# chlhnu/DOT-SOCP

Hardware: AMD Instinct MI355X
Metric: ADMM iters/sec on NxNxT dot2d staggered grid at 1/2/4/8 MI355X (higher is better)
Workload: dtype f64

## Files before the change

dot-socp_amd/capi.py:

```python
import ctypes
import os

import numpy as np

_HERE = os.path.dirname(os.path.abspath(__file__))
LIB_PATH = os.path.join(_HERE, "lib", "libdotsocp.so")

i64 = ctypes.c_longlong
dbl = ctypes.c_double
vp = ctypes.c_void_p


class DotsocpError(RuntimeError):
    def __init__(self, code, msg):
        super().__init__(f"libdotsocp error {code}: {msg}")
        self.code = code


class Problem(ctypes.Structure):
    _fields_ = [("dim", ctypes.c_int), ("weighted", ctypes.c_int),
                ("ny", i64), ("nx", i64), ("nt", i64),
                ("D", dbl), ("E", dbl), ("cScale", dbl), ("dScale", dbl),
                ("normc", dbl), ("normd", dbl)]


class Opts(ctypes.Structure):
    _fields_ = [("tau", dbl), ("sigma", dbl), ("tol", dbl), ("maxit", i64),
                ("ifCheckStepByStep", ctypes.c_int), ("checkPrimDualFeas", ctypes.c_int),
                ("scaling", ctypes.c_int), ("time_limit", dbl)]


class Result(ctypes.Structure):
    _fields_ = [("sigma", dbl), ("sigma_internal", dbl), ("cScale", dbl), ("dScale", dbl),
                ("times", dbl * 7), ("iters", i64), ("hist_len", i64), ("stopped", ctypes.c_int),
                ("time_extra", dbl)]


class AccOpts(ctypes.Structure):
    _fields_ = [("restart", i64), ("rho", dbl), ("theta", dbl)]


REPORT_BINS = 49
REPORT_RHO_FLOOR = 1e-8


class Report(ctypes.Structure):
    _fields_ = [("n_nodes", i64), ("n_cells", i64), ("mass_err", dbl), ("neg_err", dbl),
                ("rho_min", dbl), ("rho_neg", i64), ("rho_hist", i64 * REPORT_BINS),
                ("fq_max", dbl), ("fq_pos", i64), ("fq_hist", i64 * REPORT_BINS),
                ("cost", dbl), ("nonfinite", i64)]


class AdvectOpts(ctypes.Structure):
    _fields_ = [("n", i64), ("nsub", ctypes.c_int), ("direction", ctypes.c_int), ("rho_floor", dbl)]


class PushOpts(ctypes.Structure):
    _fields_ = [("n", i64), ("nsub", ctypes.c_int), ("direction", ctypes.c_int), ("rho_floor", dbl), ("nf", i64)]


class MapReport(ctypes.Structure):
    _fields_ = [("n", i64), ("n_clamped", i64), ("n_still", i64), ("mass", dbl),
                ("cost_map", dbl), ("cost_length", dbl), ("cost_action", dbl), ("disp_mean", dbl), ("len_mean", dbl),
                ("disp_max", dbl), ("len_max", dbl), ("detour_max", dbl),
                ("detour_hist", i64 * REPORT_BINS), ("detour_over", i64)]


class RenderOpts(ctypes.Structure):
    _fields_ = [("mode", ctypes.c_int), ("channels", ctypes.c_int), ("nf", i64), ("nlevels", ctypes.c_int),
                ("barrier_index", ctypes.c_int), ("vmax", dbl), ("skip_y", i64), ("skip_x", i64), ("mask_frac", dbl)]


class RenderInfo(ctypes.Structure):
    _fields_ = [("vmax", dbl), ("rho_min", dbl), ("nonfinite", i64), ("masked", i64), ("my", i64), ("mx", i64)]


RENDER_LINEAR, RENDER_INVERTED, RENDER_LEVELS = 0, 1, 2
METHOD_INPALM, METHOD_PALM, METHOD_ACCADMM = 0, 1, 2


F_PHI, F_Q, F_ALPHA, F_Z, F_BETA, F_C, F_WEIGHT = range(7)

SYMBOLS = {
    "dotsocp_last_error": (ctypes.c_char_p, []),
    "dotsocp_version": (ctypes.c_char_p, []),
    "dotsocp_device_count": (ctypes.c_int, []),
    "dotsocp_proj_soc": (ctypes.c_int, [vp, vp, i64, i64]),
    "dotsocp_bfd": (ctypes.c_int, [vp, vp, i64, i64, i64, dbl, dbl]),
    "dotsocp_bfd_conj": (ctypes.c_int, [vp, vp, i64, i64, i64, dbl]),
    "dotsocp_bfd1d": (ctypes.c_int, [vp, vp, i64, i64, dbl, dbl]),
    "dotsocp_bfd_conj1d": (ctypes.c_int, [vp, vp, i64, i64, dbl]),
    "dotsocp_oper_poisson": (ctypes.c_int, [vp, vp, i64, i64, i64, dbl]),
    "dotsocp_dctn": (ctypes.c_int, [vp, i64, i64, i64, ctypes.c_int]),
    "dotsocp_proj_soc_dev": (ctypes.c_int, [vp, vp, i64, i64, vp]),
    "dotsocp_bfd_dev": (ctypes.c_int, [vp, vp, i64, i64, i64, dbl, dbl, vp]),
    "dotsocp_bfd_conj_dev": (ctypes.c_int, [vp, vp, i64, i64, i64, dbl, vp]),
    "dotsocp_create": (vp, [ctypes.POINTER(Problem), ctypes.c_int, ctypes.c_int]),
    "dotsocp_create_multi": (vp, [ctypes.POINTER(Problem), ctypes.c_int, ctypes.c_int]),
    "dotsocp_destroy": (None, [vp]),
    "dotsocp_rccl_unique_id": (ctypes.c_int, [vp]),
    "dotsocp_attach_rccl": (ctypes.c_int, [vp, vp, ctypes.c_int, ctypes.c_int]),
    "dotsocp_slab_range": (ctypes.c_int, [i64, ctypes.c_int, ctypes.c_int, ctypes.POINTER(i64), ctypes.POINTER(i64)]),
    "dotsocp_field_len": (i64, [ctypes.POINTER(Problem), ctypes.c_int]),
    "dotsocp_dct_algorithm": (ctypes.c_int, [i64]),
    "dotsocp_dct_levels": (ctypes.c_int, [i64, ctypes.c_int]),
    "dotsocp_cdft_levels": (ctypes.c_int, [i64]),
    "dotsocp_tsolve_tri_safe": (ctypes.c_int, [i64, i64, i64]),
    "dotsocp_cone_writes_beta": (ctypes.c_int, [i64, dbl, i64, ctypes.c_int, ctypes.c_int, ctypes.c_int, dbl, dbl]),
    "dotsocp_rescale_due": (ctypes.c_int, [i64, ctypes.c_int, dbl, dbl]),
    "dotsocp_qcone_form": (ctypes.c_int, [i64, dbl, i64, ctypes.c_int, ctypes.c_int, ctypes.c_int, ctypes.c_int, dbl, dbl]),
    "dotsocp_release_cache": (i64, []),
    "dotsocp_upload": (ctypes.c_int, [vp, ctypes.c_int, vp]),
    "dotsocp_upload_layers": (ctypes.c_int, [vp, ctypes.c_int, vp, i64, i64]),
    "dotsocp_download": (ctypes.c_int, [vp, ctypes.c_int, vp]),
    "dotsocp_begin": (ctypes.c_int, [vp, ctypes.POINTER(Opts)]),
    "dotsocp_begin_method": (ctypes.c_int, [vp, ctypes.POINTER(Opts), ctypes.c_int, ctypes.POINTER(AccOpts)]),
    "dotsocp_run": (ctypes.c_int, [vp, i64, ctypes.POINTER(i64)]),
    "dotsocp_recover_outputs": (ctypes.c_int, [vp, vp, vp, vp, vp, vp, vp, vp, vp]),
    "dotsocp_report_edges": (ctypes.c_int, [vp]),
    "dotsocp_solution_report": (ctypes.c_int, [vp, vp, vp, ctypes.POINTER(Report), vp, vp]),
    "dotsocp_recover_velocity": (ctypes.c_int, [vp, vp, vp, dbl, vp, vp]),
    "dotsocp_advect_particles": (ctypes.c_int, [vp, vp, vp, ctypes.POINTER(AdvectOpts), vp, vp, vp, vp, ctypes.POINTER(i64)]),
    "dotsocp_push_mass": (ctypes.c_int, [vp, vp, vp, ctypes.POINTER(PushOpts), vp, vp, vp, vp, vp, ctypes.POINTER(i64),
                                         ctypes.POINTER(dbl), vp]),
    "dotsocp_map_report": (ctypes.c_int, [vp, vp, vp, ctypes.POINTER(AdvectOpts), vp, vp, vp, ctypes.POINTER(MapReport),
                                          vp, vp, vp]),
    "dotsocp_render_evolution": (ctypes.c_int, [vp, vp, vp, ctypes.POINTER(RenderOpts), vp, vp, vp, vp, vp, vp, vp,
                                                ctypes.POINTER(RenderInfo)]),
    "dotsocp_jump_next_level": (ctypes.c_int, [vp, vp]),
    "dotsocp_finish": (ctypes.c_int, [vp, ctypes.POINTER(Result)]),
    "dotsocp_get_history": (ctypes.c_int, [vp, vp, vp, vp, vp]),
    "dotsocp_set_profiling": (ctypes.c_int, [vp, ctypes.c_int]),
    "dotsocp_kernel_time": (ctypes.c_int, [vp, ctypes.c_char_p, ctypes.POINTER(dbl), ctypes.POINTER(i64)]),
    "dotsocp_canary_check": (ctypes.c_int, []),
    "dotsocp_poisson_phi": (ctypes.c_int, [vp]),
    "dotsocp_synchronize": (ctypes.c_int, [vp]),
    "dotsocp_weights_create": (vp, [ctypes.c_int, i64, i64, i64, ctypes.c_int]),
    "dotsocp_weights_destroy": (None, [vp]),
    "dotsocp_weights_len": (i64, [i64, i64, i64, ctypes.c_int, ctypes.c_int]),
    "dotsocp_weights_set": (ctypes.c_int, [vp, vp]),
    "dotsocp_weights_set_space": (ctypes.c_int, [vp, vp, vp]),
    "dotsocp_weights_restrict": (ctypes.c_int, [vp, ctypes.c_int]),
    "dotsocp_weights_log10_mean": (ctypes.c_int, [vp, ctypes.c_int, ctypes.POINTER(dbl)]),
    "dotsocp_weights_download": (ctypes.c_int, [vp, ctypes.c_int, vp]),
    "dotsocp_upload_weight_from": (ctypes.c_int, [vp, vp, ctypes.c_int]),
}

_lib = None


def _share_torchs_hip_runtime():
    import importlib.util
    import sys
    if "torch" in sys.modules or os.environ.get("DOTSOCP_SYSTEM_HIP"):
        return
    try:
        spec = importlib.util.find_spec("torch")
    except (ImportError, ValueError):
        return
    if not spec or not spec.submodule_search_locations:
        return
    for name in ("libamdhip64.so", "libamdhip64.so.7"):
        path = os.path.join(list(spec.submodule_search_locations)[0], "lib", name)
        if os.path.exists(path):
            try:
                ctypes.CDLL(path, mode=ctypes.RTLD_GLOBAL)
            except OSError:
                pass
            return


def lib():
    global _lib
    if _lib is None:
        _share_torchs_hip_runtime()
        if not os.path.exists(LIB_PATH):
            raise ImportError(
                f"{LIB_PATH} is missing: build the HIP extension first "
                "(python -c 'import __graft_entry__ as g; g.build()'); there is no CPU fallback")
        L = ctypes.CDLL(LIB_PATH)
        for name, (res, args) in SYMBOLS.items():
            f = getattr(L, name)
            f.restype = res
            f.argtypes = args
        _lib = L
    return _lib


def check(code):
    if code != 0:
        raise DotsocpError(code, lib().dotsocp_last_error().decode())


def fptr(a):
    if not isinstance(a, np.ndarray) or a.dtype != np.float64 or not (a.flags.f_contiguous or a.flags.c_contiguous):
        raise ValueError("expected a contiguous float64 numpy array")
    return a.ctypes.data


def slab_range(nt, world, rank):
    t0, t1 = i64(), i64()
    check(lib().dotsocp_slab_range(nt, world, rank, ctypes.byref(t0), ctypes.byref(t1)))
    return t0.value, t1.value


def rccl_unique_id():
    buf = (ctypes.c_ubyte * 128)()
    check(lib().dotsocp_rccl_unique_id(buf))
    return bytes(buf)


DCT_ALGORITHMS = ("none", "fft", "pfa", "rader", "bluestein", "dense")


def dct_algorithm(n):
    return DCT_ALGORITHMS[lib().dotsocp_dct_algorithm(int(n))]


def dct_levels(n, axis):
    return int(lib().dotsocp_dct_levels(int(n), int(axis)))


def cdft_levels(n):
    return int(lib().dotsocp_cdft_levels(int(n)))
```

dot-socp_amd/csrc/capi.hip:

```cpp
#include <cstring>
#include <new>

#include "comm.h"
#include "solver.h"
#include "weights.h"

using namespace dotsocp;

namespace dotsocp {
extern thread_local std::string g_last_error;
int dotsocp_slab_range_impl(i64 nt, int world, int rank, i64 *t0, i64 *t1);
}

struct dotsocp_ctx {
    Solver s;
};

struct dotsocp_weights {
    Weights w;
};

static int require_device() {
    int n = 0;
    if (hipGetDeviceCount(&n) != hipSuccess || n <= 0) {
        set_error("no HIP device available (libdotsocp has no CPU fallback)");
        return DOTSOCP_ENODEVICE;
    }
    return 0;
}

struct DevBuf {
    double *p = nullptr;
    ~DevBuf() { dfree(p); }
    int alloc(i64 n) { return dmalloc(&p, n); }
};

extern "C" {

const char *dotsocp_last_error(void) { return g_last_error.c_str(); }
const char *dotsocp_version(void) { return "dotsocp-mi355x 0.1 (gfx950)"; }

int dotsocp_device_count(void) {
    int n = 0;
    if (hipGetDeviceCount(&n) != hipSuccess) return 0;
    return n;
}

int dotsocp_proj_soc_dev(double *d_out, const double *d_in, dotsocp_i64 M, dotsocp_i64 K, void *stream) {
    DS_ARG(M >= 0 && K >= 2, "mexProjSoc needs an M x K matrix with K >= 2");
    DS_ARG(d_out && d_in, "NULL pointer");
    return launch_proj_soc(d_out, d_in, M, K, (hipStream_t)stream);
}

static int make_grid(Grid &g, i64 nt, i64 nx, i64 ny) {
    DS_ARG(nt >= 2 && nx >= 1 && ny >= 1, "need nt >= 2, nx >= 1, ny >= 1");
    g.set(ny, nx, nt, 0, nt);
    return 0;
}

int dotsocp_bfd_dev(double *d_z, const double *d_q, dotsocp_i64 nt, dotsocp_i64 nx, dotsocp_i64 ny, double scale,
                    double dF, void *stream) {
    Grid g;
    DS_CHECK(make_grid(g, nt, nx, ny));
    DS_ARG(d_z && d_q, "NULL pointer");
    return launch_bfd(g, d_z, d_q, scale, dF, (hipStream_t)stream);
}

int dotsocp_bfd_conj_dev(double *d_q, const double *d_z, dotsocp_i64 nt, dotsocp_i64 nx, dotsocp_i64 ny,
                         double scale, void *stream) {
    Grid g;
    DS_CHECK(make_grid(g, nt, nx, ny));
    DS_ARG(d_z && d_q, "NULL pointer");
    return launch_bfd_conj(g, d_q, d_z, scale, (hipStream_t)stream);
}

int dotsocp_proj_soc(double *out, const double *in, dotsocp_i64 M, dotsocp_i64 K) {
    DS_ARG(M >= 0 && K >= 2, "mexProjSoc needs an M x K matrix with K >= 2");
    if (M == 0) return 0;
    DS_ARG(out && in, "NULL pointer");
    DS_CHECK(require_device());
    DevBuf a, b;
    DS_CHECK(a.alloc(M * K));
    DS_CHECK(b.alloc(M * K));
    DS_HIP(hipMemcpy(a.p, in, sizeof(double) * M * K, hipMemcpyHostToDevice));
    DS_CHECK(launch_proj_soc(b.p, a.p, M, K, nullptr));
    DS_HIP(hipDeviceSynchronize());
    DS_HIP(hipMemcpy(out, b.p, sizeof(double) * M * K, hipMemcpyDeviceToHost));
    return 0;
}

int dotsocp_bfd(double *z, const double *q, dotsocp_i64 nt, dotsocp_i64 nx, dotsocp_i64 ny, double scale,
                double dF) {
    Grid g;
    DS_CHECK(make_grid(g, nt, nx, ny));
    DS_ARG(z && q, "NULL pointer");
    DS_CHECK(require_device());
    DevBuf dz, dq;
    DS_CHECK(dz.alloc(10 * g.Nz));
    DS_CHECK(dq.alloc(g.NqAlloc));
    DS_HIP(hipMemcpy(dz.p, z, sizeof(double) * 10 * g.Nz, hipMemcpyHostToDevice));
    DS_HIP(hipMemcpy(dq.p, q, sizeof(double) * g.NqAlloc, hipMemcpyHostToDevice));
    DS_CHECK(launch_bfd(g, dz.p, dq.p, scale, dF, nullptr));
    DS_HIP(hipDeviceSynchronize());
    DS_HIP(hipMemcpy(z, dz.p, sizeof(double) * 10 * g.Nz, hipMemcpyDeviceToHost));
    return 0;
}

int dotsocp_bfd_conj(double *q, const double *z, dotsocp_i64 nt, dotsocp_i64 nx, dotsocp_i64 ny, double scale) {
    Grid g;
    DS_CHECK(make_grid(g, nt, nx, ny));
    DS_ARG(z && q, "NULL pointer");
    DS_CHECK(require_device());
    DevBuf dz, dq;
    DS_CHECK(dz.alloc(10 * g.Nz));
    DS_CHECK(dq.alloc(g.NqAlloc));
    DS_HIP(hipMemcpy(dz.p, z, sizeof(double) * 10 * g.Nz, hipMemcpyHostToDevice));
    DS_CHECK(launch_bfd_conj(g, dq.p, dz.p, scale, nullptr));
    DS_HIP(hipDeviceSynchronize());
    DS_HIP(hipMemcpy(q, dq.p, sizeof(double) * g.NqAlloc, hipMemcpyDeviceToHost));
    return 0;
}

static const int k1dCols[6] = {0, 5, 6, 7, 8, 9};

int dotsocp_bfd1d(double *z, const double *q, dotsocp_i64 nt, dotsocp_i64 nx, double scale, double dF) {
    Grid g;
    DS_CHECK(make_grid(g, nt, 1, nx));
    DS_ARG(z && q, "NULL pointer");
    DS_CHECK(require_device());
    DevBuf dz, dq;
    DS_CHECK(dz.alloc(10 * g.Nz));
    DS_CHECK(dq.alloc(g.NqAlloc));
    for (int j = 0; j < 6; ++j)
        DS_HIP(hipMemcpy(dz.p + k1dCols[j] * g.Nz, z + j * g.Nz, sizeof(double) * g.Nz, hipMemcpyHostToDevice));
    DS_HIP(hipMemcpy(dq.p, q, sizeof(double) * g.NqAlloc, hipMemcpyHostToDevice));
    DS_CHECK(launch_bfd(g, dz.p, dq.p, scale, dF, nullptr));
    DS_HIP(hipDeviceSynchronize());
    for (int j = 0; j < 6; ++j)
        DS_HIP(hipMemcpy(z + j * g.Nz, dz.p + k1dCols[j] * g.Nz, sizeof(double) * g.Nz, hipMemcpyDeviceToHost));
    return 0;
}

int dotsocp_bfd_conj1d(double *q, const double *z, dotsocp_i64 nt, dotsocp_i64 nx, double scale) {
    Grid g;
    DS_CHECK(make_grid(g, nt, 1, nx));
    DS_ARG(z && q, "NULL pointer");
    DS_CHECK(require_device());
    DevBuf dz, dq;
    DS_CHECK(dz.alloc(10 * g.Nz));
    DS_CHECK(dq.alloc(g.NqAlloc));
    DS_HIP(hipMemset(dz.p, 0, sizeof(double) * 10 * g.Nz));
    for (int j = 0; j < 6; ++j)
        DS_HIP(hipMemcpy(dz.p + k1dCols[j] * g.Nz, z + j * g.Nz, sizeof(double) * g.Nz, hipMemcpyHostToDevice));
    DS_CHECK(launch_bfd_conj(g, dq.p, dz.p, scale, nullptr));
    DS_HIP(hipDeviceSynchronize());
    DS_HIP(hipMemcpy(q, dq.p, sizeof(double) * g.NqAlloc, hipMemcpyDeviceToHost));
    return 0;
}

static int dctn_dev(double *a, double *b, i64 ny, i64 nx, i64 nt, int inverse, DctPlan *py, DctPlan *px, DctPlan *pt) {
    if (!inverse) {
        DS_CHECK(launch_dct_axis(py, a, b, ny, nx, nt, 0, 0, nullptr));
        DS_CHECK(launch_dct_axis(px, b, a, ny, nx, nt, 1, 0, nullptr));
        DS_CHECK(launch_dct_axis(pt, a, b, ny, nx, nt, 2, 0, nullptr));
    } else {
        DS_CHECK(launch_dct_axis(pt, a, b, ny, nx, nt, 2, 1, nullptr));
        DS_CHECK(launch_dct_axis(px, b, a, ny, nx, nt, 1, 1, nullptr));
        DS_CHECK(launch_dct_axis(py, a, b, ny, nx, nt, 0, 1, nullptr));
    }
    return 0;
}

struct Plans {
    DctPlan *py = nullptr, *px = nullptr, *pt = nullptr;
    ~Plans() { dct_plan_destroy(py); dct_plan_destroy(px); dct_plan_destroy(pt); }
    int make(i64 ny, i64 nx, i64 nt) {
        DS_CHECK(dct_length_check(ny)); DS_CHECK(dct_length_check(nx)); DS_CHECK(dct_length_check(nt));
        py = dct_plan_create(ny); px = dct_plan_create(nx); pt = dct_plan_create(nt);
        if (!py || !px || !pt) { set_error("DCT plan allocation failed"); return DOTSOCP_EHIP; }
        return 0;
    }
};

int dotsocp_dctn(double *a, dotsocp_i64 ny, dotsocp_i64 nx, dotsocp_i64 nt, int inverse) {
    DS_ARG(a && ny >= 1 && nx >= 1 && nt >= 1, "bad array");
    DS_CHECK(dct_length_check(ny)); DS_CHECK(dct_length_check(nx)); DS_CHECK(dct_length_check(nt));
    DS_CHECK(require_device());
    const i64 n = ny * nx * nt;
    DevBuf da, db;
    Plans pl;
    DS_CHECK(da.alloc(n));
    DS_CHECK(db.alloc(n));
    DS_CHECK(pl.make(ny, nx, nt));
    DS_HIP(hipMemcpy(da.p, a, sizeof(double) * n, hipMemcpyHostToDevice));
    DS_CHECK(dctn_dev(da.p, db.p, ny, nx, nt, inverse, pl.py, pl.px, pl.pt));
    DS_HIP(hipDeviceSynchronize());
    DS_HIP(hipMemcpy(a, db.p, sizeof(double) * n, hipMemcpyDeviceToHost));
    return 0;
}

int dotsocp_oper_poisson(double *res, const double *rhs, dotsocp_i64 ny, dotsocp_i64 nx, dotsocp_i64 nt,
                         double kernelScale) {
    DS_ARG(res && rhs && ny >= 1 && nx >= 1 && nt >= 1, "bad array");
    DS_CHECK(dct_length_check(ny)); DS_CHECK(dct_length_check(nx)); DS_CHECK(dct_length_check(nt));
    DS_CHECK(require_device());
    const i64 n = ny * nx * nt;
    DevBuf da, db, cy, cx, ct;
    Plans pl;
    DS_CHECK(da.alloc(n));
    DS_CHECK(db.alloc(n));
    DS_CHECK(pl.make(ny, nx, nt));
    const double pi = 3.14159265358979323846;
    auto table = [&](DevBuf &d, i64 m) -> int {
        std::vector<double> t((size_t)m);
        for (i64 k = 0; k < m; ++k) t[k] = (2.0 * (double)(m - 1) * (double)(m - 1)) * (1.0 - cos(pi * (double)k / (double)m));
        DS_CHECK(d.alloc(m));
        DS_HIP(hipMemcpy(d.p, t.data(), sizeof(double) * m, hipMemcpyHostToDevice));
        return 0;
    };
    DS_CHECK(table(cy, ny));
    DS_CHECK(table(cx, nx));
    DS_CHECK(table(ct, nt));
    DS_HIP(hipMemcpy(da.p, rhs, sizeof(double) * n, hipMemcpyHostToDevice));
    Grid g;
    g.set(ny, nx, nt, 0, nt);
    DS_CHECK(launch_dct_axis(pl.py, da.p, db.p, ny, nx, nt, 0, 0, nullptr));
    DS_CHECK(launch_dct_axis(pl.px, db.p, da.p, ny, nx, nt, 1, 0, nullptr));
    DS_CHECK(launch_poisson_t_single(pl.pt, g, kernelScale, cy.p, cx.p, ct.p, da.p, db.p, 0, nullptr, tsolve_tri_allowed()));
    DS_CHECK(launch_dct_axis(pl.px, da.p, db.p, ny, nx, nt, 1, 1, nullptr));
    DS_CHECK(launch_dct_axis(pl.py, db.p, da.p, ny, nx, nt, 0, 1, nullptr));
    DS_HIP(hipDeviceSynchronize());
    DS_HIP(hipMemcpy(res, da.p, sizeof(double) * n, hipMemcpyDeviceToHost));
    return 0;
}

dotsocp_ctx *dotsocp_create(const dotsocp_problem *prob, int device, int nslabs) {
    dotsocp_ctx *c = new (std::nothrow) dotsocp_ctx();
    if (!c) { set_error("out of host memory"); return nullptr; }
    if (c->s.init(prob, device, nslabs) != 0) {
        delete c;
        return nullptr;
    }
    return c;
}

dotsocp_ctx *dotsocp_create_multi(const dotsocp_problem *prob, int first_device, int ngpu) {
    dotsocp_ctx *c = new (std::nothrow) dotsocp_ctx();
    if (!c) { set_error("out of host memory"); return nullptr; }
    if (c->s.init(prob, first_device, ngpu, true) != 0) {
        delete c;
        return nullptr;
    }
    return c;
}

void dotsocp_destroy(dotsocp_ctx *ctx) { delete ctx; }

int dotsocp_slab_range(dotsocp_i64 nt, int world, int rank, dotsocp_i64 *t0, dotsocp_i64 *t1) {
    DS_ARG(t0 && t1 && world >= 1 && rank >= 0 && rank < world && nt >= 2 * world, "bad slab request");
    return dotsocp_slab_range_impl(nt, world, rank, t0, t1);
}

int dotsocp_rccl_unique_id(unsigned char id[128]) {
    DS_ARG(id != nullptr, "id is NULL");
    Rccl &api = rccl_api();
    DS_CHECK(api.load());
    ncclUniqueId uid;
    static_assert(sizeof(uid) == 128, "ncclUniqueId is expected to be 128 bytes");
    DS_NCCL(api.GetUniqueId(&uid));
    memcpy(id, &uid, sizeof uid);
    return 0;
}

int dotsocp_attach_rccl(dotsocp_ctx *ctx, const unsigned char id[128], int rank, int world) {
    if (!ctx) { set_error("ctx is NULL"); return DOTSOCP_EINVAL; }
    return ctx->s.attach_rccl(id, rank, world);
}

#define CTX_OR_FAIL()                                      \
    do {                                                   \
        if (!ctx) { set_error("ctx is NULL"); return DOTSOCP_EINVAL; } \
        (void)hipGetLastError();    \
    } while (0)

int dotsocp_dct_algorithm(dotsocp_i64 n) { return dct_choose_algorithm(n); }
int dotsocp_dct_levels(dotsocp_i64 n, int axis) { return dct_levels(n, axis); }
int dotsocp_cdft_levels(dotsocp_i64 n) { return cdft_levels(n); }
int dotsocp_tsolve_tri_safe(dotsocp_i64 ny, dotsocp_i64 nx, dotsocp_i64 nt) { return tsolve_tri_safe(ny, nx, nt) ? 1 : 0; }

int dotsocp_cone_writes_beta(dotsocp_i64 it, double last_sigma_it, dotsocp_i64 maxit, int check_step_by_step,
                             int last_of_run, int rescale, double maxFeas, double relGap) {
    return cone_writes_beta(it, last_sigma_it, maxit, check_step_by_step != 0, last_of_run != 0, rescale, maxFeas, relGap) ? 1 : 0;
}
int dotsocp_rescale_due(dotsocp_i64 it, int rescale, double maxFeas, double relGap) {
    return rescale_due(it, rescale, maxFeas, relGap) ? 1 : 0;
}
int dotsocp_qcone_form(dotsocp_i64 it, double last_sigma_it, dotsocp_i64 maxit, int check_step_by_step, int last_of_run,
                       int next_last_of_run, int rescale, double maxFeas, double relGap) {
    return qcone_form(it, last_sigma_it, maxit, check_step_by_step != 0, last_of_run != 0, next_last_of_run != 0, rescale,
                      maxFeas, relGap);
}

dotsocp_i64 dotsocp_field_len(const dotsocp_problem *p, int field) {
    if (!p || (p->dim != 1 && p->dim != 2) || p->nt < 2 || p->nx < 1 || (p->dim == 2 && p->ny < 1)) return -1;
    const i64 ny = p->dim == 1 ? p->nx : p->ny, nx = p->dim == 1 ? 1 : p->nx, nt = p->nt;
    const i64 Nphi = ny * nx * nt, Nz = ny * nx * (nt - 1);
    const i64 Nq = Nz + ny * (nx - 1) * nt + (ny - 1) * nx * nt;
    switch (field) {
        case DOTSOCP_F_PHI: case DOTSOCP_F_C: return Nphi;
        case DOTSOCP_F_Q: case DOTSOCP_F_ALPHA: case DOTSOCP_F_WEIGHT: return Nq;
        case DOTSOCP_F_Z: case DOTSOCP_F_BETA: return Nz * (p->dim == 1 ? 6 : 10);
        default: return -1;
    }
}

int dotsocp_upload(dotsocp_ctx *ctx, int field, const double *host) { CTX_OR_FAIL(); return ctx->s.upload(field, host); }
dotsocp_i64 dotsocp_release_cache(void) { return (dotsocp_i64)device_cache_release(); }

int dotsocp_upload_layers(dotsocp_ctx *ctx, int field, const double *host, dotsocp_i64 t0, dotsocp_i64 n) {
    CTX_OR_FAIL();
    return ctx->s.upload_layers(field, host, t0, n);
}
int dotsocp_download(dotsocp_ctx *ctx, int field, double *host) { CTX_OR_FAIL(); return ctx->s.download(field, host); }
int dotsocp_begin(dotsocp_ctx *ctx, const dotsocp_opts *opts) { CTX_OR_FAIL(); return ctx->s.begin(opts); }
int dotsocp_begin_method(dotsocp_ctx *ctx, const dotsocp_opts *opts, int method, const dotsocp_acc_opts *acc) {
    CTX_OR_FAIL();
    return ctx->s.begin_method(opts, method, acc);
}
int dotsocp_recover_outputs(dotsocp_ctx *ctx, const double *rho0, const double *rho1, double *rho, double *Ex,
                            double *Ey, double *q0, double *bx, double *by) {
    CTX_OR_FAIL();
    if (ctx->s.prob.dim == 1)
        return ctx->s.recover_outputs(rho0, rho1, rho, nullptr, Ex, q0, nullptr, bx);
    return ctx->s.recover_outputs(rho0, rho1, rho, Ex, Ey, q0, bx, by);
}

int dotsocp_report_edges(double edges[DOTSOCP_REPORT_BINS + 1]) {
    if (!edges) { set_error("invalid argument: report_edges() needs an array of %d doubles", DOTSOCP_REPORT_BINS + 1); return DOTSOCP_EINVAL; }
    report_edges_host(edges);
    return 0;
}

int dotsocp_solution_report(dotsocp_ctx *ctx, const double *rho0, const double *rho1, dotsocp_report *rep, double *layer_mass,
                            double *layer_neg) {
    CTX_OR_FAIL();
    return ctx->s.solution_report(rho0, rho1, rep, layer_mass, layer_neg);
}

int dotsocp_recover_velocity(dotsocp_ctx *ctx, const double *rho0, const double *rho1, double rho_floor, double *vx, double *vy) {
    CTX_OR_FAIL();
    if (ctx->s.prob.dim == 1)
        return ctx->s.recover_velocity(rho0, rho1, rho_floor, nullptr, vx);
    return ctx->s.recover_velocity(rho0, rho1, rho_floor, vx, vy);
}

int dotsocp_advect_particles(dotsocp_ctx *ctx, const double *rho0, const double *rho1, const dotsocp_advect_opts *o, double *x,
                             double *y, double *traj_x, double *traj_y, dotsocp_i64 *n_clamped) {
    CTX_OR_FAIL();
    if (ctx->s.prob.dim == 1)
        return ctx->s.advect_particles(rho0, rho1, o, nullptr, x, nullptr, traj_x, n_clamped);
    return ctx->s.advect_particles(rho0, rho1, o, x, y, traj_x, traj_y, n_clamped);
}

int dotsocp_push_mass(dotsocp_ctx *ctx, const double *rho0, const double *rho1, const dotsocp_push_opts *o, double *x, double *y,
                      const double *mass, const dotsocp_i64 *frame_nodes, double *frames, dotsocp_i64 *n_clamped, double *unit,
                      double *l1) {
    CTX_OR_FAIL();
    if (ctx->s.prob.dim == 1)
        return ctx->s.push_mass(rho0, rho1, o, nullptr, x, mass, frame_nodes, frames, n_clamped, unit, l1);
    return ctx->s.push_mass(rho0, rho1, o, x, y, mass, frame_nodes, frames, n_clamped, unit, l1);
}

int dotsocp_map_report(dotsocp_ctx *ctx, const double *rho0, const double *rho1, const dotsocp_advect_opts *o, double *x, double *y,
                       const double *mass, dotsocp_map_report_t *rep, double *disp, double *len, double *action) {
    CTX_OR_FAIL();
    if (ctx->s.prob.dim == 1)
        return ctx->s.map_report(rho0, rho1, o, nullptr, x, mass, rep, disp, len, action);
    return ctx->s.map_report(rho0, rho1, o, x, y, mass, rep, disp, len, action);
}

int dotsocp_render_evolution(dotsocp_ctx *ctx, const double *rho0, const double *rho1, const dotsocp_render_opts *opts,
                             const dotsocp_i64 *frame_nodes, const double *levels, const unsigned char *lut,
                             const unsigned char *barrier, unsigned char *image, double *mvx, double *mvy,
                             dotsocp_render_info *info) {
    CTX_OR_FAIL();
    if (ctx->s.prob.dim != 1 || !opts)
        return ctx->s.render_evolution(rho0, rho1, opts, frame_nodes, levels, lut, barrier, image, mvx, mvy, info);
    dotsocp_render_opts o = *opts;
    if (o.skip_y >= 1 && o.skip_x >= 1) { o.skip_y = o.skip_x; o.skip_x = 1; }
    dotsocp_render_info got{};
    const int rc = ctx->s.render_evolution(rho0, rho1, &o, frame_nodes, levels, lut, barrier, image, nullptr, mvx, &got);
    if (rc == 0 && info) {
        *info = got;
        info->mx = got.my;
        info->my = got.my > 0 ? 1 : 0;
    }
    return rc;
}

int dotsocp_jump_next_level(dotsocp_ctx *coarse, dotsocp_ctx *fine) {
    if (!coarse || !fine) { set_error("context is NULL"); return DOTSOCP_EINVAL; }
    return fine->s.jump_from(coarse->s);
}

int dotsocp_run(dotsocp_ctx *ctx, dotsocp_i64 n_iters, dotsocp_i64 *done) { CTX_OR_FAIL(); return ctx->s.run(n_iters, done); }
int dotsocp_finish(dotsocp_ctx *ctx, dotsocp_result *res) { CTX_OR_FAIL(); return ctx->s.finish(res); }

int dotsocp_get_history(dotsocp_ctx *ctx, double *kkt, double *time, double *iter, double *pdGap) {
    CTX_OR_FAIL();
    const Solver &s = ctx->s;
    const size_t n = s.hist_iter.size();
    for (size_t i = 0; i < n; ++i) {
        if (kkt) for (int j = 0; j < 7; ++j) kkt[j * n + i] = s.hist_kkt[i * 7 + j];
        if (time) time[i] = s.hist_time[i];
        if (iter) iter[i] = s.hist_iter[i];
        if (pdGap) pdGap[i] = s.hist_gap[i];
    }
    return 0;
}

int dotsocp_set_profiling(dotsocp_ctx *ctx, int on) {
    CTX_OR_FAIL();
    ctx->s.profiling = on != 0;
    return 0;
}

int dotsocp_kernel_time(dotsocp_ctx *ctx, const char *name, double *avg_ms, dotsocp_i64 *launches) {
    CTX_OR_FAIL();
    DS_ARG(name != nullptr, "name is NULL");
    static const char *names[PH_COUNT] = {"rhs", "poisson", "cone_proj", "qstep", "beta", "kkt",
                                          "cone_fused_a", "cone_fused_b", "materialise", "comm",
                                          "interp", "acc_cone", "acc_gather", "qstep_first", "transpose", "cone_carry", "qcone",
                                          "velocity_layer", "advect", "deposit", "frame_l1", "advect_path", "map_final"};
    for (int i = 0; i < PH_COUNT; ++i)
        if (strcmp(name, names[i]) == 0) {
            const i64 n = ctx->s.phase_launches[i];
            if (avg_ms) *avg_ms = n ? ctx->s.phase_ms[i] / (double)n : 0.0;
            if (launches) *launches = n;
            return 0;
        }
    set_error("unknown kernel family '%s'", name);
    return DOTSOCP_EINVAL;
}

int dotsocp_canary_check(void) {
    std::string rep;
    const int bad = canary_check(&rep);
    if (bad) set_error("canary: %d device buffer(s) written out of bounds: %s", bad, rep.c_str());
    return bad;
}

#define WEIGHTS_OR_FAIL()                                  \
    do {                                                   \
        if (!w) { set_error("weight pyramid is NULL"); return DOTSOCP_EINVAL; } \
        (void)hipGetLastError();                           \
    } while (0)

dotsocp_weights *dotsocp_weights_create(int device, dotsocp_i64 ny, dotsocp_i64 nx, dotsocp_i64 nt, int levels) {
    dotsocp_weights *w = new (std::nothrow) dotsocp_weights();
    if (!w) { set_error("out of host memory"); return nullptr; }
    if (w->w.init(device, ny, nx, nt, levels) != 0) {
        delete w;
        return nullptr;
    }
    return w;
}

void dotsocp_weights_destroy(dotsocp_weights *w) { delete w; }

dotsocp_i64 dotsocp_weights_len(dotsocp_i64 ny, dotsocp_i64 nx, dotsocp_i64 nt, int levels, int level) {
    return weights_level_len(ny, nx, nt, levels, level);
}

int dotsocp_weights_set(dotsocp_weights *w, const double *weight) { WEIGHTS_OR_FAIL(); return w->w.set(weight); }
int dotsocp_weights_set_space(dotsocp_weights *w, const double *weightX, const double *weightY) {
    WEIGHTS_OR_FAIL();
    return w->w.set_space(weightX, weightY);
}
int dotsocp_weights_restrict(dotsocp_weights *w, int log_mean) { WEIGHTS_OR_FAIL(); return w->w.restrict_all(log_mean); }
int dotsocp_weights_log10_mean(dotsocp_weights *w, int level, double *mean) { WEIGHTS_OR_FAIL(); return w->w.log10_mean(level, mean); }
int dotsocp_weights_download(dotsocp_weights *w, int level, double *host) { WEIGHTS_OR_FAIL(); return w->w.download(level, host); }

int dotsocp_upload_weight_from(dotsocp_ctx *ctx, dotsocp_weights *w, int level) {
    CTX_OR_FAIL();
    WEIGHTS_OR_FAIL();
    const Weights::Level *L = nullptr;
    DS_CHECK(w->w.level_for_upload(level, &L));
    return ctx->s.upload_weight_from(L->w, w->w.device, L->ny, L->nx, L->nt);
}

int dotsocp_poisson_phi(dotsocp_ctx *ctx) { CTX_OR_FAIL(); return ctx->s.poisson_phi(); }

int dotsocp_synchronize(dotsocp_ctx *ctx) {
    CTX_OR_FAIL();
    ctx->s.cur_dev = -1;
    return ctx->s.sync_all();
}

}
```

dot-socp_amd/csrc/fused.hip:

```cpp
#include "device_utils.h"
#include "gather_tile.h"
#include "kernels.h"

#include <cstdlib>

namespace dotsocp {

template <int MODE, int XB, bool NT = false, bool GIN = false, bool GOUT = false>
__global__ void __launch_bounds__(64 * XB) k_cone_fused(Grid g, LoopCoef c, FusedArgs a) {
    static_assert(MODE == 1 || !(GIN || GOUT), "the gamma form exists between two MODE_B passes only");
    constexpr bool DUAL = (MODE >= 5);
    constexpr bool UPD = (MODE != 0 && MODE != 6);
    constexpr bool PROJ = (MODE < 2 || MODE >= 5);
    __shared__ double2 xch[2][XB][64];
    __shared__ double2 xchp[DUAL ? 2 : 1][DUAL ? XB : 1][DUAL ? 64 : 1];
    const int lane = threadIdx.x, xl = threadIdx.y;
    const BlockId blk = block_id(a.xcd != 0);
    const i64 y = (i64)blk.x * 64 + lane;
    const i64 x = (i64)blk.y * XB + xl;
    const bool inb = (y < g.ny) && (x < g.nx);
    const i64 yc = inb ? y : 0, xc = inb ? x : 0;
    const i64 t0 = ((i64)blk.z + a.z0) * a.TC;
    const i64 t1 = (t0 + a.TC < g.ncl) ? t0 + a.TC : g.ncl;
    const bool lastChunk = (t1 == g.ncl);
    constexpr bool GATHER = (PROJ || MODE == 4);
    const bool carried = GATHER && !DUAL && t0 > 0 && a.carry_in != nullptr;
    const i64 tstart = (GATHER && t0 > 0 && !carried) ? t0 - 1 : t0;
    const i64 nxblk = gridDim.y, nyblk = gridDim.x;

    EdgeQuad cur = load_edges(g, a.q, yc, xc, tstart, c.sf), curo, cur3;
    if (UPD && !GIN) curo = load_edges(g, a.q_old, yc, xc, tstart, c.sf);
    if (MODE == 5) cur3 = load_edges(g, a.q3, yc, xc, tstart, c.sf);
    GatherCarry gc, gcp;
    if (carried) {
        const i64 ci = yc + g.py * xc;
        gc.p3 = a.carry_in[ci]; gc.p4 = a.carry_in[g.plane + ci];
        gc.p7 = a.carry_in[2 * g.plane + ci]; gc.p8 = a.carry_in[3 * g.plane + ci];
    }
    const i64 tstop = (GATHER && lastChunk) ? t1 + 1 : t1;
    for (i64 tl = tstart; tl < tstop; ++tl) {
        const bool hasCell = tl < g.ncl;
        const bool own = tl >= t0;
        double w[10], wp[10];
        if (hasCell) {
            const i64 i = yc + g.py * (xc + g.nx * tl);
            const EdgeQuad nxt = load_edges(g, a.q, yc, xc, tl + 1, c.sf);
            double b[10], v[10];
#pragma unroll
            for (int j = 0; j < 10; ++j) b[j] = ld_stream<NT>(a.beta_in + j * g.Nc + i);
            if (!GIN) apply_scale_ops(b, a.bops);
            build_z2(v, a.q[i], cur, nxt, c.s, c.dF);
            if constexpr (GIN) {
#pragma unroll
                for (int j = 0; j < 10; ++j) b[j] = mult_finish(b[j], v[j], c.tau);
                if (!GOUT && own && inb) {
#pragma unroll
                    for (int j = 0; j < 10; ++j) st_stream<NT>(a.beta_out + j * g.Nc + i, b[j]);
                }
            } else if constexpr (UPD) {
                const EdgeQuad nxto = load_edges(g, a.q_old, yc, xc, tl + 1, c.sf);
                double zo[10];
                build_z2(zo, a.q_old[i], curo, nxto, c.s, c.dF);
#pragma unroll
                for (int j = 0; j < 10; ++j) zo[j] = zo[j] - b[j];
                proj_row<10>(zo);
#pragma unroll
                for (int j = 0; j < 10; ++j) b[j] = mult_finish(mult_carry(b[j], zo[j], c.tau), v[j], c.tau);
                if (own && inb) {
                    if (MODE != 3 && !GOUT) {
#pragma unroll
                        for (int j = 0; j < 10; ++j) st_stream<NT>(a.beta_out + j * g.Nc + i, b[j]);
                    }
                    if (MODE == 2 || MODE == 3) {
#pragma unroll
                        for (int j = 0; j < 10; ++j) st_stream<NT>(a.z_out + j * g.Nc + i, zo[j]);
                    }
                }
                curo = nxto;
                if (MODE == 4) {
#pragma unroll
                    for (int j = 0; j < 10; ++j) w[j] = zo[j] + b[j];
                    if (own && inb) a.q2[i] = c.s * (w[9] - w[0]);
                }
            }
            cur = nxt;
            if (PROJ) {
                if (MODE == 5) {
                    const EdgeQuad nxt3 = load_edges(g, a.q3, yc, xc, tl + 1, c.sf);
                    build_z2(v, a.q3[i], cur3, nxt3, c.s, c.dF);
                    cur3 = nxt3;
                }
#pragma unroll
                for (int j = 0; j < 10; ++j) v[j] = v[j] - b[j];
                proj_row<10>(v);
                if (GOUT && own && inb) {
#pragma unroll
                    for (int j = 0; j < 10; ++j) st_stream<NT>(a.beta_out + j * g.Nc + i, mult_carry(b[j], v[j], c.tau));
                }
#pragma unroll
                for (int j = 0; j < 10; ++j) w[j] = v[j] + b[j];
                if (own && inb) a.q2[i] = c.s * (w[9] - w[0]);
                if (DUAL) {
#pragma unroll
                    for (int j = 0; j < 10; ++j) wp[j] = w[j] + c.tau * v[j];
                    if (own && inb) a.p2[i] = c.s * (wp[9] - wp[0]);
                }
            }
        } else {
#pragma unroll
            for (int j = 0; j < 10; ++j) w[j] = 0.0;
            if (DUAL) {
#pragma unroll
                for (int j = 0; j < 10; ++j) wp[j] = 0.0;
            }
        }
        if constexpr (GATHER && !DUAL)
            gather_emit<XB>(g, c.sf, xch, gc, w, tl, own && inb, x, y, xl, lane, nxblk, nyblk, blk.y, blk.x,
                            a.q2, a.sx, a.sy);
        if constexpr (DUAL) {
            gather_post<XB>(xch, gc, w, xl, lane);
            gather_post<XB>(xchp, gcp, wp, xl, lane);
            __syncthreads();
            gather_finish<XB>(g, c.sf, xch, gc, w, tl, own && inb, x, y, xl, lane, nxblk, nyblk, blk.y, blk.x,
                              a.q2, a.sx, a.sy);
            gather_finish<XB>(g, c.sf, xchp, gcp, wp, tl, own && inb, x, y, xl, lane, nxblk, nyblk, blk.y, blk.x,
                              a.p2, a.sxp, a.syp);
        }
    }
    if (GATHER && !DUAL && !lastChunk && a.carry_out != nullptr && inb) {
        const i64 ci = y + g.py * x;
        a.carry_out[ci] = gc.p3; a.carry_out[g.plane + ci] = gc.p4;
        a.carry_out[2 * g.plane + ci] = gc.p7; a.carry_out[3 * g.plane + ci] = gc.p8;
    }
}

bool stream_nt_enabled() {
    const char *e = getenv("DOTSOCP_NT");
    return !(e && atoi(e) == 0);
}

bool tile_xcd_remap(const Grid &g) {
    return (g.py % 16) != 0;
}

bool cone_split_enabled() { return true; }

int fused_geometry(const Grid &g, FusedGeom &fg) {
    fg.XB = 4;
    fg.nyblk = (g.ny + 63) / 64;
    fg.nxblk = (g.nx + fg.XB - 1) / fg.XB;
    const i64 tiles = fg.nyblk * fg.nxblk;
    const i64 target = 2048;
    i64 chunks = (target + tiles - 1) / tiles;
    if (chunks < 1) chunks = 1;
    if (!(g.first && g.last) && cone_split_enabled() && chunks < 2 && g.ncl >= 12) chunks = 2;
    i64 TC = (g.ncl + chunks - 1) / chunks;
    if (TC < 8) TC = 8;
    if (TC > g.ncl) TC = g.ncl;
    if (TC < 1) TC = 1;
    fg.TC = TC;
    fg.chunks = (g.ncl + TC - 1) / TC;
    fg.sx_len = (g.ncl + 1) * fg.nxblk * g.ny;
    fg.sy_len = (g.ncl + 1) * g.nx * fg.nyblk;
    return 0;
}

int launch_cone_fused(int mode, const Grid &g, const LoopCoef &c, const FusedGeom &fg, FusedArgs a,
                      hipStream_t st, i64 z0, i64 zcount, int flavour) {
    if (g.Nz <= 0) return 0;
    if (zcount < 0) zcount = fg.chunks - z0;
    if (z0 < 0 || zcount <= 0 || z0 + zcount > fg.chunks) return 0;
    a.TC = fg.TC;
    a.z0 = (int)z0;
    a.xcd = tile_xcd_remap(g) ? 1 : 0;
    dim3 grid((unsigned)fg.nyblk, (unsigned)fg.nxblk, (unsigned)zcount);
    dim3 blk(64, 4);
    const bool nt = stream_nt_enabled();
#define CONE_MODE(M)                                                                     \
    case M:                                                                              \
        if (nt) DS_KLAUNCH((k_cone_fused<M, 4, true>), grid, blk, 0, st, g, c, a);       \
        else DS_KLAUNCH((k_cone_fused<M, 4>), grid, blk, 0, st, g, c, a);                \
        break;
    if (flavour != 0) {
        if (mode != 1 || (flavour & ~(CONE_GIN | CONE_GOUT))) { set_error("bad fused flavour"); return DOTSOCP_EINVAL; }
        if ((flavour & CONE_GIN) && !a.bops.empty()) { set_error("internal: gamma with a pending scaling"); return DOTSOCP_ESTATE; }
#define CONE_FLAV(GI, GO)                                                                          \
        if (nt) DS_KLAUNCH((k_cone_fused<1, 4, true, GI, GO>), grid, blk, 0, st, g, c, a);         \
        else DS_KLAUNCH((k_cone_fused<1, 4, false, GI, GO>), grid, blk, 0, st, g, c, a);
        if (flavour == CONE_GOUT) { CONE_FLAV(false, true) }
        else if (flavour == CONE_GIN) { CONE_FLAV(true, false) }
        else { CONE_FLAV(true, true) }
#undef CONE_FLAV
        DS_HIP(hipGetLastError());
        return 0;
    }
    switch (mode) {
        CONE_MODE(0) CONE_MODE(1) CONE_MODE(2) CONE_MODE(3) CONE_MODE(4) CONE_MODE(5) CONE_MODE(6)
#undef CONE_MODE
        default: set_error("bad fused mode"); return DOTSOCP_EINVAL;
    }
    DS_HIP(hipGetLastError());
    return 0;
}

}
```

dot-socp_amd/csrc/kernels.h:

```cpp
#pragma once
#include "common.h"
#include "defer.h"
#include "particle_block.h"

namespace dotsocp {

struct LoopCoef {
    double s;
    double sf;
    double dF;
    double at, ax, ay;
    double tau;
    double c1, c2;
    double dinv1, dinv2;
};

enum {
    S_Q2 = 0, S_Z2, S_APHI2, S_ALPHA2, S_BETA2, S_FBBETA2, S_PRIM1, S_PRIM2, S_DUAL1, S_DUAL2,
    S_COMPLEM, S_DOTCOMP, S_RHO2, S_RHOFQ2, S_MRHOB, S_M2, S_RHOB2, S_QALPHA, S_CPHI, S_PHI2,
    S_COUNT
};

struct KktCoef {
    double sigma;
    double kappa;
    double dsD;
    double dsE;
};

struct ScaleOps {
    int n;
    double mul, div;
    double mul2, div2;
    bool empty() const { return n == 0; }
    void clear() { n = 0; }
    bool push(double m, double d) {
        if (n >= 2) return false;
        if (n == 0) { mul = m; div = d; } else { mul2 = m; div2 = d; }
        n += 1;
        return true;
    }
};

int launch_proj_soc(double *out, const double *in, i64 M, i64 K, hipStream_t st);
int launch_bfd(const Grid &g, double *z, const double *q, double s, double dF, hipStream_t st);
int launch_bfd_conj(const Grid &g, double *q, const double *w, double s, hipStream_t st, const double *tail_bx = nullptr,
                    const double *tail_by = nullptr);
int launch_cone_proj(const Grid &g, const LoopCoef &c, const double *q, const double *beta, double *z,
                     hipStream_t st);
int launch_beta_update(const Grid &g, const LoopCoef &c, const double *q, const double *z, double *beta,
                       hipStream_t st);
int launch_gather_tail(const Grid &g, const double *z, const double *beta, double *tail_bx, double *tail_by,
                       hipStream_t st);

struct FusedGeom {
    int XB;
    i64 nyblk, nxblk;
    i64 TC, chunks;
    i64 sx_len, sy_len;
};
struct FusedArgs {
    const double *q_old;
    const double *q;
    const double *beta_in;
    double *beta_out;
    double *z_out;
    double *q2;
    double *sx, *sy;
    const double *q3;
    double *p2, *sxp, *syp;
    i64 TC;
    ScaleOps bops;
    int xcd;
    int z0;
    const double *carry_in;
    double *carry_out;
};
bool tile_xcd_remap(const Grid &g);
int fused_geometry(const Grid &g, FusedGeom &fg);
enum { CONE_GIN = 1, CONE_GOUT = 2 };
int launch_cone_fused(int mode, const Grid &g, const LoopCoef &c, const FusedGeom &fg, FusedArgs a,
                      hipStream_t st, i64 z0 = 0, i64 zcount = -1, int flavour = 0);
bool cone_split_enabled();

struct KktWork;
struct AccArgs {
    const double *q;
    const double *z_in, *beta_in;
    const double *z0, *beta0;
    double *z0_out, *beta0_out;
    double bdiv;
    KktCoef kk;
    const double *alpha_p, *weight;
    double *partials;
    int nostore;
    double *z_out, *beta_out;
    double *q2, *sx, *sy;
    i64 TC;
    double c1, c2, om_rho, rho;
};
struct AccCoef {
    double c1, c2, om_rho, rho;
    double om_c1, c1c2;
};
int launch_acc_cone(int mode, const Grid &g, const LoopCoef &c, const FusedGeom &fg, AccArgs a, hipStream_t st);
int launch_acc_cone_kkt(const Grid &g, const LoopCoef &c, const FusedGeom &fg, AccArgs a, const KktWork &w, hipStream_t st);
int launch_acc_restart(double *x, const double *xp, double *anchor, i64 n, const AccCoef &k, double div, hipStream_t st);
int launch_acc_interp(double *x, const double *xp, double *aux, i64 n, const AccCoef &k, int mode, int write_aux,
                      hipStream_t st);

int launch_prolong_phi(const Grid &gf, const Grid &gc, const double *phic, double *phif, double sc_in, double sc_out,
                       hipStream_t st, i64 tc0 = 0);
int launch_prolong_beta(const Grid &gf, const Grid &gc, const double *betac, double *betaf, double *neg, double sc_in0,
                        double sc_in1, double sc_out, hipStream_t st, i64 tc0 = 0, i64 Nzc = -1);
int launch_scale_div(double *x, const double *w, i64 n, double sc, hipStream_t st);
int launch_fill(double *x, i64 n, double v, hipStream_t st);
int launch_outputs(const Grid &g, const double *q, const double *alpha, const double *weight, const double *rho0,
                   const double *rho1, const double *a_prev, double sig, double cD, double dD, int which, double *out,
                   hipStream_t st);
int launch_out_tail(const Grid &g, const double *alpha, const double *weight, double sig, double cD, double *out,
                    hipStream_t st);

int launch_velocity_layer(const Grid &g, const double *alpha, const double *weight, const double *rho0, const double *rho1,
                          const double *a_prev, double sig, double cD, bool dim1, i64 tl, double floor, double *vX, double *vY,
                          hipStream_t st);
int launch_advect_seed(bool dim1, i64 n, double *px, double *py, unsigned int *flag, hipStream_t st);
int launch_advect(bool dim1, i64 ny, i64 nx, i64 py, const double *vX0, const double *vY0, const double *vX1,
                  const double *vY1, i64 n, int nsub, int dir, double dt, double *px, double *py_, unsigned int *flag,
                  hipStream_t st, double *sq = nullptr, double *len = nullptr);
int launch_advect_count(const unsigned int *flag, i64 n, unsigned long long *count, hipStream_t st);
int launch_deposit(bool dim1, i64 ny, i64 nx, i64 py, i64 n, const double *px, const double *py_, const i64 *units,
                   unsigned long long *cnt, hipStream_t st);
int launch_frame_l1(const Grid &g, const double *alpha, const double *weight, const double *rho0, const double *rho1,
                    const double *a_prev, double sig, double cD, i64 tl, double unit, double *frame, double *partials,
                    double *sum, hipStream_t st);
i64 map_blocks(i64 n);
int launch_map_final(bool dim1, i64 n, const double *px, const double *py_, const double *sq, const double *len, const double *sx,
                     const double *sy, const double *mass, const double *edges, double steps, double *disp, double *action,
                     double *partials, double *sums, unsigned long long *counts, hipStream_t st);

enum { RC_RHO_HIST = 0, RC_FQ_HIST = DOTSOCP_REPORT_BINS, RC_RHO_NEG = 2 * DOTSOCP_REPORT_BINS, RC_FQ_POS, RC_NONFINITE,
       RC_RHO_MIN, RC_FQ_MAX, RC_COUNT };
void report_edges_host(double edges[DOTSOCP_REPORT_BINS + 1]);
double report_key_decode(unsigned long long key, bool inverted, double none);
i64 report_tiles(const Grid &g);
int launch_report_rows(const double *partials, i64 tiles, i64 rows, double *sums, hipStream_t st);
int launch_report(const Grid &g, const double *q, const double *alpha, const double *weight, const double *rho0,
                  const double *rho1, const double *a_prev, double sig, double cD, double dD, bool dim1, const double *edges,
                  double *partials, double *sums, unsigned long long *counts, hipStream_t st);

enum { RR_MAX = 0, RR_MIN, RR_NONFINITE, RR_MASKED, RR_COUNT };
#define RND_LEVELS 255
int launch_rho_range(const Grid &g, const double *alpha, const double *weight, const double *rho0, const double *rho1,
                     const double *a_prev, double sig, double cD, const unsigned char *barrier, unsigned long long *counts,
                     hipStream_t st);
int launch_render(const Grid &g, const double *alpha, const double *weight, const double *rho0, const double *rho1,
                  const double *a_prev, double sig, double cD, i64 tl, int mode, int channels, const unsigned char *barrier,
                  const double *levels, int nlevels, const unsigned char *lut, int barrier_index, double vmax,
                  unsigned char *image, hipStream_t st);
int launch_movement(const Grid &g, const double *alpha, const double *weight, const double *rho0, const double *rho1,
                    const double *a_prev, double sig, double cD, i64 tl, i64 skip_y, i64 skip_x, i64 my, i64 mx, double thr,
                    double *mvX, double *mvY, hipStream_t st);

struct QStepExtra {
    ScaleOps aops;
    double *partials, *resid;
    double kappa, dsD;
    double *u0_tail;
    int c_ends;
};
int launch_qstep_rhs(const Grid &g, const LoopCoef &c, const FusedGeom &fg, const double *phi, const double *q2,
                     const double *sx, const double *sy, const double *weight, const double *tail_bx,
                     const double *tail_by, const double *cvec, double *q_out, const double *alpha_in, double *alpha_out,
                     double *rhs, hipStream_t st, i64 z0 = 0, i64 zcount = -1, i64 zstride = 1,
                     const QStepExtra *ex = nullptr);
i64 qstep_rhs_blocks(const Grid &g, const FusedGeom &fg);
struct QConeArgs {
    const double *phi, *q2v, *sx, *sy, *cvec, *alpha_in, *gamma_in;
    double *alpha_out, *rhs, *q_out, *beta_out, *q2_out, *sx_out, *sy_out;
    i64 TC;
    int ap_on;
    double ap_mul, ap_div;
    int c_ends;
};
int launch_qcone(const Grid &g, const LoopCoef &c, const FusedGeom &fg, QConeArgs a, bool gout, hipStream_t st);
i64 qcone_chunk_len(const Grid &g);
i64 qstep_rhs_chunks(const Grid &g, const FusedGeom &fg, i64 *TC = nullptr);
int launch_qstep_rhs_acc(int var, const Grid &g, const LoopCoef &c, const FusedGeom &fg, const double *phi,
                         const double *q2, const double *sx, const double *sy, const double *weight, const double *cvec,
                         double *q_raw, const double *alpha_in, double *alpha_out, double *rhs, double *q_state,
                         const double *q_anchor, const double *alpha_anchor, const AccCoef &k, hipStream_t st,
                         const double *tail_bx = nullptr, const double *tail_by = nullptr, double *u0_tail = nullptr);
int launch_qstep_palm_first(const Grid &g, const LoopCoef &c, const FusedGeom &fg, const double *phi, const double *q2,
                            const double *sx, const double *sy, const double *cvec, double *q_out, const double *alpha,
                            double *rhs, hipStream_t st, const double *tail_bx = nullptr, const double *tail_by = nullptr,
                            const double *qk = nullptr);

int launch_qstep_fused(const Grid &g, const LoopCoef &c, const FusedGeom &fg, const double *phi,
                       const double *q2, const double *sx, const double *sy, const double *weight,
                       const double *tail_bx, const double *tail_by, double *q_out, double *alpha,
                       hipStream_t st);
int launch_rhs_sigma_fix(const Grid &g, double *rhs, const double *r, double *cvec, double factor, hipStream_t st,
                         bool c_ends = false);
int launch_c_interior_test(const Grid &g, const double *cvec, int *flag, hipStream_t st);
int launch_rhs_fixup(const Grid &g, const LoopCoef &c, const double *u0_prev, double *rhs, hipStream_t st);
int launch_grad(const Grid &g, const LoopCoef &c, const double *phi, double *out, hipStream_t st);
int launch_tail_finalize(const Grid &g, const LoopCoef &c, const FusedGeom &fg, const double *q2, const double *sx,
                         const double *sy, double *tail_bx, double *tail_by, hipStream_t st);
int launch_kkt_tail(const Grid &g, const double *alpha, const double *beta, const double *weight, double *a0,
                    double *a0w, double *bt_bx, double *bt_by, hipStream_t st);
int launch_rhs(const Grid &g, const LoopCoef &c, const double *q, const double *alpha, const double *cvec,
               const double *weight, const double *u0_prev, double *rhs, hipStream_t st, bool c_ends = false);
int launch_qstep(const Grid &g, const LoopCoef &c, const double *phi, const double *z, const double *beta,
                 const double *weight, const double *tail_bx, const double *tail_by, double *q,
                 double *alpha, hipStream_t st);
int launch_u0_tail(const Grid &g, const double *q, const double *alpha, const double *weight, double *out,
                   hipStream_t st);
int launch_scale(double *x, i64 n, double mul, double div, hipStream_t st);
#define DS_MAX_WORLD 64
struct PencilCuts {
    int world;
    i64 cut[DS_MAX_WORLD + 1];
};
int launch_pencil_pack(bool pack, const PencilCuts &pc, i64 plane, i64 ntl, double *slab, double *stage, hipStream_t st);

#define TRI_EXTRA 256
int launch_tri_local(const Grid &g, i64 nt, double kscale, const double *cy, const double *cx, const PencilCuts &pc,
                     const double *r, double *send, hipStream_t st);
int launch_tri_reduced(const Grid &g, i64 nt, double kscale, const double *cy, const double *cx, const PencilCuts &pc,
                       int rank, i64 l0, i64 nl, const i64 *slab_n, const double *recv, double *back, double *zero_work,
                       hipStream_t st, const double *own_recv = nullptr, double *own_back = nullptr);
int launch_tri_final(const Grid &g, i64 nt, double kscale, const double *cy, const double *cx, const PencilCuts &pc,
                     const double *back, double *x, hipStream_t st);
bool tsolve_tri_supported(i64 nt);
bool tsolve_tri_preferred(i64 nt, bool pow2, i64 plane);
bool tsolve_tri_safe(i64 ny, i64 nx, i64 nt);
int launch_tsolve_tri(const Grid &g, i64 nt, double kscale, const double *cy, const double *cx, double *x, hipStream_t st);
int device_cus();
struct GatherMsgs {
    const double *src[DS_MAX_WORLD];
    double *dst[DS_MAX_WORLD];
    i64 count[DS_MAX_WORLD];
    int n;
};
int launch_gather_msgs(const GatherMsgs &m, hipStream_t st);

#define KKT_SLICES 64
struct KktWork {
    double *partials;
    i64 maxBlocks;
    double *sums;
};
struct KktHalo {
    const double *a0_prev, *a0w_prev, *btail_bx, *btail_by;
};
i64 kkt_partials_needed(const Grid &g);
int launch_kkt(const Grid &g, const LoopCoef &c, const KktCoef &k, const double *phi, const double *q,
               const double *alpha, const double *z, const double *beta, const double *cvec,
               const double *weight, const KktHalo &halo, const KktWork &w, int parts, hipStream_t st,
               bool layer0 = false, double *resid = nullptr);
int launch_kkt_nodual(const Grid &g, const LoopCoef &c, const KktCoef &k, const double *phi, const double *q,
                      const double *alpha, const double *cvec, const double *weight, const KktWork &w, hipStream_t st);
int launch_kkt_bnd_dual(const Grid &g, const LoopCoef &c, const KktCoef &k, const FusedGeom &fg, const double *q,
                        const double *alpha, const double *weight, const double *q2, const double *sx, const double *sy,
                        const KktWork &w, hipStream_t st);
int launch_kkt_cells_update(const Grid &g, const LoopCoef &c, const KktCoef &k, const FusedGeom &fg, FusedArgs a,
                            const double *phi, const double *alpha, const double *weight, const KktWork &w,
                            hipStream_t st, bool edges = false, const double *q_new = nullptr);
int launch_norms(const Grid &g, const LoopCoef &c, const KktCoef &k, const FusedGeom &fg, FusedArgs a, const double *phi,
                 const double *alpha, const double *weight, const KktWork &w, hipStream_t st);
double *kkt_qstep_partials(const Grid &g, const KktWork &w);
int launch_kkt_final(const Grid &g, const KktWork &w, hipStream_t st);

enum { DCT_ALG_NONE = 0, DCT_ALG_FFT = 1, DCT_ALG_PFA = 2, DCT_ALG_RADER = 3, DCT_ALG_BLUESTEIN = 4, DCT_ALG_DENSE = 5 };
int dct_choose_algorithm(i64 n);
struct DctPlan;
int dct_levels(i64 n, int axis);
int dct_length_check(i64 n);
int cdft_levels(i64 n);
DctPlan *dct_plan_create(i64 n);
void dct_plan_destroy(DctPlan *p);
int launch_dct_axis(const DctPlan *p, const double *src, double *dst, i64 n0, i64 n1, i64 n2, int axis,
                    int inverse, hipStream_t st, i64 pitch0 = 0);
bool dct_plan_is_pow2(const DctPlan *p);
bool dct_plan_has_tsolve(const DctPlan *p);
int launch_dct_t_solve(const DctPlan *p, const double *src, double *dst, i64 ny, i64 nplane, i64 line0, i64 nl,
                       i64 nt, double kscale, const double *cy, const double *cx, const double *ct, hipStream_t st,
                       i64 pitch0 = 0);
int launch_spectral_divide_pencil(double *data, i64 ny, i64 line0, i64 nl, i64 nt, double kscale, const double *cy,
                                  const double *cx, const double *ct, hipStream_t st);
int launch_spectral_divide(double *data, i64 ny, i64 nt, i64 x0, i64 nxl, double kscale, const double *cy,
                           const double *cx, const double *ct, hipStream_t st, i64 pitch0 = 0);
bool tsolve_tri_allowed();
int launch_poisson_t_single(const DctPlan *pt, const Grid &g, double kscale, const double *cy, const double *cx,
                            const double *ct, double *p, double *p2, i64 pitch0, hipStream_t st, bool allow_tri);

}
```

dot-socp_amd/csrc/kkt.hip:

```cpp
#include "device_utils.h"
#include "gather_tile.h"
#include "kernels.h"

#include <cstdlib>

namespace dotsocp {

struct WBeta {
    const double *b;
    i64 Nz;
    __device__ __forceinline__ double operator()(int j, i64 cell) const { return b[j * Nz + cell]; }
};

template <bool WEIGHTED, int PART, bool NODUAL = false>
__global__ void __launch_bounds__(TILE_Y *TILE_X) k_kkt(Grid g, LoopCoef c, KktCoef k, i64 chunk,
                                                         const double *__restrict__ phi, const double *__restrict__ q,
                                                         const double *__restrict__ alpha, const double *__restrict__ z,
                                                         const double *__restrict__ beta,
                                                         const double *__restrict__ cvec,
                                                         const double *__restrict__ weight,
                                                         KktHalo halo, double *__restrict__ partials,
                                                         double *__restrict__ resid) {
    const i64 y = (i64)blockIdx.x * TILE_Y + threadIdx.x;
    const i64 x = (i64)blockIdx.y * TILE_X + threadIdx.y;
    const bool inb = (y < g.ny) && (x < g.nx);
    const i64 tbeg = (i64)blockIdx.z * chunk;
    const i64 tend = (tbeg + chunk < g.ntl) ? tbeg + chunk : g.ntl;
    double S[S_COUNT];
#pragma unroll
    for (int i = 0; i < S_COUNT; ++i) S[i] = 0.0;
    WBeta WB{beta, g.Nc};
    auto wgt = [&](i64 idx) { return WEIGHTED ? weight[idx] : 1.0; };
    auto rhoT_at = [&](i64 yy, i64 xx, i64 tl) -> double {
        if (tl >= g.ncl) return 0.0;
        if (tl < 0) {
            if (g.first) return 0.0;
            return k.kappa * halo.a0w_prev[yy + g.py * xx];
        }
        const i64 cidx = yy + g.py * (xx + g.nx * tl);
        return k.kappa * (wgt(cidx) * alpha[cidx]);
    };
    auto rho_node = [&](i64 yy, i64 xx, i64 tl) { return (rhoT_at(yy, xx, tl - 1) + rhoT_at(yy, xx, tl)) / 2.0; };
    auto edge_sums = [&](i64 idx, double tmp, double q2b) {
        const double w = wgt(idx);
        const double qv = q[idx], av = alpha[idx];
        const double wq = w * qv, wa = w * av;
        S[S_Q2] += qv * qv;
        S[S_ALPHA2] += av * av;
        S[S_APHI2] += tmp * tmp;
        const double r1 = tmp - wq;
        S[S_PRIM1] += r1 * r1;
        if (!NODUAL) {
            S[S_FBBETA2] += q2b * q2b;
            const double r2 = q2b + wa;
            S[S_DUAL2] += r2 * r2;
        }
        S[S_QALPHA] += wq * av;
    };
    if (inb) {
        for (i64 tl = tbeg; tl < tend; ++tl) {
            const i64 node = y + g.py * (x + g.nx * tl);
            const i64 bxo = g.offBx + g.bxLayer * tl, byo = g.offBy + g.byLayer * tl;
            if (PART & 1) {
                double r = 0.0;
                if (tl >= 1)
                    r += c.at * alpha[node - g.plane];
                else if (!g.first)
                    r += c.at * halo.a0_prev[y + g.py * x];
                if (tl < g.ncl) r += (-c.at) * alpha[node];
                if (x >= 1) r += c.ax * alpha[bxo + y + g.py * (x - 1)];
                if (x <= g.nx - 2) r += (-c.ax) * alpha[bxo + y + g.py * x];
                if (y >= 1) r += c.ay * alpha[byo + (y - 1) + g.pyb * x];
                if (y <= g.ny - 2) r += (-c.ay) * alpha[byo + y + g.pyb * x];
                const double cv = cvec[node], pv = phi[node];
                r = r - cv;
                if (resid) resid[node] = (tl == 0 && !g.first) ? r - c.at * halo.a0_prev[y + g.py * x] : r;
                S[S_DUAL1] += r * r;
                S[S_CPHI] += cv * pv;
                S[S_PHI2] += pv * pv;
            }
            if ((PART & 2) && tl < g.ncl) {
                const EdgeQuad ea = load_edges(g, q, y, x, tl, c.sf);
                const EdgeQuad eb = load_edges(g, q, y, x, tl + 1, c.sf);
                const double q0 = q[node];
                double z2[10], zz[10], p[10];
                build_z2(z2, q0, ea, eb, c.s, c.dF);
                double zs = 0.0, bs = 0.0, rs = 0.0;
#pragma unroll
                for (int j = 0; j < 10; ++j) {
                    const double zv = z[j * g.Nc + node], bv = beta[j * g.Nc + node];
                    zz[j] = zv;
                    p[j] = zv - k.sigma * bv;
                    zs += zv * zv;
                    bs += bv * bv;
                    const double d = zv - z2[j];
                    rs += d * d;
                }
                proj_row<10>(p);
                double cs = 0.0;
#pragma unroll
                for (int j = 0; j < 10; ++j) {
                    const double d = zz[j] - p[j];
                    cs += d * d;
                }
                S[S_Z2] += zs;
                S[S_BETA2] += bs;
                S[S_PRIM2] += rs;
                S[S_COMPLEM] += cs;
                const double rhoT = rhoT_at(y, x, tl);
                double sq = 0.0;
#pragma unroll
                for (int j = 1; j < 9; ++j) {
                    const double e = k.dsE * z2[j];
                    sq += e * e;
                }
                double rhoFq = rhoT + k.dsD * q0 + sq / 4.0;
                rhoFq = (rhoFq < 0.0) ? 0.0 : rhoFq;
                const double dd = rhoT - rhoFq;
                S[S_DOTCOMP] += dd * dd;
                S[S_RHO2] += rhoT * rhoT;
                S[S_RHOFQ2] += rhoFq * rhoFq;
                double tmp = (-c.at) * phi[node];
                tmp += c.at * phi[node + g.plane];
                edge_sums(node, tmp, c.s * (WB(9, node) - WB(0, node)));
            }
            if ((PART & 16) && tl < g.ncl) {
                double tmp = (-c.at) * phi[node];
                tmp += c.at * phi[node + g.plane];
                edge_sums(node, tmp, 0.0);
            }
            if ((PART & 4) && x < g.nx - 1) {
                const i64 idx = bxo + y + g.py * x;
                double tmp = (-c.ax) * phi[node];
                tmp += c.ax * phi[node + g.py];
                const double q2b = NODUAL ? 0.0 : c.sf * gather_bx(g, WB, y, x, tl, halo.btail_bx);
                edge_sums(idx, tmp, q2b);
                const double rm = (rho_node(y, x, tl) + rho_node(y, x + 1, tl)) / 2.0;
                const double rb = k.dsD * (rm * q[idx]);
                const double m = k.kappa * (wgt(idx) * alpha[idx]);
                const double d = m - rb;
                S[S_MRHOB] += d * d;
                S[S_M2] += m * m;
                S[S_RHOB2] += rb * rb;
            }
            if ((PART & 8) && y < g.ny - 1) {
                const i64 idx = byo + y + g.pyb * x;
                double tmp = (-c.ay) * phi[node];
                tmp += c.ay * phi[node + 1];
                const double q2b = NODUAL ? 0.0 : c.sf * gather_by(g, WB, y, x, tl, halo.btail_by);
                edge_sums(idx, tmp, q2b);
                const double rm = (rho_node(y, x, tl) + rho_node(y + 1, x, tl)) / 2.0;
                const double rb = k.dsD * (rm * q[idx]);
                const double m = k.kappa * (wgt(idx) * alpha[idx]);
                const double d = m - rb;
                S[S_MRHOB] += d * d;
                S[S_M2] += m * m;
                S[S_RHOB2] += rb * rb;
            }
        }
    }
    __shared__ double red[TILE_X][S_COUNT];
    const int lane = threadIdx.x;
#pragma unroll
    for (int i = 0; i < S_COUNT; ++i) {
        double v = S[i];
#pragma unroll
        for (int off = 32; off >= 1; off >>= 1) v += __shfl_down(v, off, 64);
        if (lane == 0) red[threadIdx.y][i] = v;
    }
    __syncthreads();
    if (threadIdx.y == 0 && lane < S_COUNT) {
        double v = red[0][lane];
#pragma unroll
        for (int wv = 1; wv < TILE_X; ++wv) v += red[wv][lane];
        const i64 b = blockIdx.x + (i64)gridDim.x * (blockIdx.y + (i64)gridDim.y * blockIdx.z);
        partials[b * S_COUNT + lane] = v;
    }
}

template <bool WEIGHTED, bool EDGES, bool NORMS = false, bool NT = false>
__global__ void __launch_bounds__(TILE_Y *TILE_X) k_kkt_cells(Grid g, LoopCoef c, KktCoef k, FusedArgs a,
                                                               const double *__restrict__ phi,
                                                               const double *__restrict__ alpha,
                                                               const double *__restrict__ weight,
                                                               double *__restrict__ partials) {
    __shared__ double2 xch[EDGES ? 2 : 1][EDGES ? TILE_X : 1][EDGES ? 64 : 1];
    const int lane = threadIdx.x, xl = threadIdx.y;
    const i64 y = (i64)blockIdx.x * TILE_Y + lane;
    const i64 x = (i64)blockIdx.y * TILE_X + xl;
    const bool inb = (y < g.ny) && (x < g.nx);
    const i64 yc = inb ? y : 0, xc = inb ? x : 0;
    const i64 t0 = (i64)blockIdx.z * a.TC;
    const i64 t1 = (t0 + a.TC < g.ncl) ? t0 + a.TC : g.ncl;
    const bool lastChunk = (t1 == g.ncl);
    const i64 tstart = (EDGES && t0 > 0) ? t0 - 1 : t0;
    const i64 tstop = (EDGES && lastChunk) ? t1 + 1 : t1;
    const i64 nxblk = gridDim.y, nyblk = gridDim.x;
    double S[S_COUNT];
#pragma unroll
    for (int i = 0; i < S_COUNT; ++i) S[i] = 0.0;
    auto wgt = [&](i64 idx) { return WEIGHTED ? weight[idx] : 1.0; };
    double p3 = 0.0, p4 = 0.0, p7 = 0.0, p8 = 0.0;
    int par = 0;
    if (inb || EDGES) {
        EdgeQuad cur = load_edges(g, a.q, yc, xc, tstart, c.sf);
        EdgeQuad curo = load_edges(g, a.q_old, yc, xc, tstart, c.sf);
        for (i64 tl = tstart; tl < tstop; ++tl) {
            const bool hasCell = tl < g.ncl;
            const bool own = (tl >= t0) && inb;
            double b[10];
            if (hasCell) {
                const i64 i = yc + g.py * (xc + g.nx * tl);
                const EdgeQuad nxt = load_edges(g, a.q, yc, xc, tl + 1, c.sf);
                const EdgeQuad nxto = load_edges(g, a.q_old, yc, xc, tl + 1, c.sf);
                const double q0 = a.q[i];
                double v[10], zo[10];
#pragma unroll
                for (int j = 0; j < 10; ++j) b[j] = ld_stream<NT>(a.beta_in + j * g.Nc + i);
                apply_scale_ops(b, a.bops);
                build_z2(v, q0, cur, nxt, c.s, c.dF);
                build_z2(zo, a.q_old[i], curo, nxto, c.s, c.dF);
#pragma unroll
                for (int j = 0; j < 10; ++j) zo[j] = zo[j] - b[j];
                proj_row<10>(zo);
                double zs = 0.0, bs = 0.0, rs = 0.0;
#pragma unroll
                for (int j = 0; j < 10; ++j) {
                    const double r = zo[j] - v[j];
                    b[j] = mult_finish(mult_carry(b[j], zo[j], c.tau), v[j], c.tau);
                    zs += zo[j] * zo[j];
                    bs += b[j] * b[j];
                    rs += r * r;
                }
                cur = nxt;
                curo = nxto;
                if (own && NORMS) {
                    S[S_Z2] += zs;
                    S[S_BETA2] += bs;
                }
                if (own && !NORMS) {
#pragma unroll
                    for (int j = 0; j < 10; ++j) st_stream<NT>(a.beta_out + j * g.Nc + i, b[j]);
                    auto xj = [&](int j) { return zo[j] - k.sigma * b[j]; };
                    const double n = sqrt(soc_norm2(xj, 10)), x0 = xj(0);
                    double cf = (x0 / n + 1.0) * 0.5;
                    cf = (cf > 1.0) ? 1.0 : cf;
                    cf = (cf < 0.0) ? 0.0 : cf;
                    const double p0 = (cf >= 1.0) ? x0 : cf * n;
                    double cs = (zo[0] - p0) * (zo[0] - p0);
#pragma unroll
                    for (int j = 1; j < 10; ++j) {
                        const double d = zo[j] - cf * xj(j);
                        cs += d * d;
                    }
                    S[S_Z2] += zs;
                    S[S_BETA2] += bs;
                    S[S_PRIM2] += rs;
                    S[S_COMPLEM] += cs;
                    const double w = wgt(i);
                    const double av = alpha[i];
                    const double rhoT = k.kappa * (w * av);
                    double sq = 0.0;
#pragma unroll
                    for (int j = 1; j < 9; ++j) {
                        const double e = k.dsE * v[j];
                        sq += e * e;
                    }
                    double rhoFq = rhoT + k.dsD * q0 + sq / 4.0;
                    rhoFq = (rhoFq < 0.0) ? 0.0 : rhoFq;
                    const double dd = rhoT - rhoFq;
                    S[S_DOTCOMP] += dd * dd;
                    S[S_RHO2] += rhoT * rhoT;
                    S[S_RHOFQ2] += rhoFq * rhoFq;
                    const double q2b = c.s * (b[9] - b[0]);
                    const double wa = w * av;
                    S[S_FBBETA2] += q2b * q2b;
                    const double r2 = q2b + wa;
                    S[S_DUAL2] += r2 * r2;
                    if (!EDGES) {
                        double tmp = (-c.at) * phi[i];
                        tmp += c.at * phi[i + g.plane];
                        const double wq = w * q0;
                        S[S_Q2] += q0 * q0;
                        S[S_ALPHA2] += av * av;
                        S[S_APHI2] += tmp * tmp;
                        const double r1 = tmp - wq;
                        S[S_PRIM1] += r1 * r1;
                        S[S_QALPHA] += wq * av;
                    }
                }
            } else {
#pragma unroll
                for (int j = 0; j < 10; ++j) b[j] = 0.0;
            }
            if (EDGES) {
                auto dual = [&](i64 e, double acc) {
                    const double gb = c.sf * acc;
                    S[S_FBBETA2] += gb * gb;
                    const double r2 = gb + wgt(e) * alpha[e];
                    S[S_DUAL2] += r2 * r2;
                };
                xch[par][xl][lane] = make_double2(b[1], p3);
                __syncthreads();
                const bool sumLayer = (tl < g.ntl) && !(tl == 0 && !g.first);
                if (own) {
                    if (x < g.nx - 1) {
                        const i64 e = g.offBx + g.bxLayer * tl + y + g.py * x;
                        if (xl < TILE_X - 1) {
                            if (sumLayer) {
                            const double2 r = xch[par][xl + 1][lane];
                            double acc = r.x + b[2];
                            acc += r.y;
                            acc += p4;
                            dual(e, acc);
                            }
                        } else {
                            a.q2[e] = b[2] + p4;
                        }
                    }
                    if (xl == 0 && x > 0) a.sx[(tl * nxblk + blockIdx.y) * g.ny + y] = b[1] + p3;
                }
                const double u5 = __shfl_down(b[5], 1, 64), u7 = __shfl_down(p7, 1, 64);
                if (own) {
                    if (y < g.ny - 1) {
                        const i64 e = g.offBy + g.byLayer * tl + y + g.pyb * x;
                        if (lane < 63) {
                            if (sumLayer) {
                                double acc = u5 + b[6];
                                acc += u7;
                                acc += p8;
                                dual(e, acc);
                            }
                        } else {
                            a.q2[e] = b[6] + p8;
                        }
                    }
                    if (lane == 0 && y > 0) a.sy[(tl * g.nx + x) * nyblk + blockIdx.x] = b[5] + p7;
                }
                p3 = b[3]; p4 = b[4]; p7 = b[7]; p8 = b[8];
                par ^= 1;
            }
        }
    }
    __shared__ double red[TILE_X][S_COUNT];
#pragma unroll
    for (int i = 0; i < S_COUNT; ++i) {
        double v = S[i];
#pragma unroll
        for (int off = 32; off >= 1; off >>= 1) v += __shfl_down(v, off, 64);
        if (lane == 0) red[threadIdx.y][i] = v;
    }
    __syncthreads();
    if (threadIdx.y == 0 && lane < S_COUNT) {
        double v = red[0][lane];
#pragma unroll
        for (int wv = 1; wv < TILE_X; ++wv) v += red[wv][lane];
        const i64 bb = blockIdx.x + (i64)gridDim.x * (blockIdx.y + (i64)gridDim.y * blockIdx.z);
        partials[bb * S_COUNT + lane] = v;
    }
}

__global__ void __launch_bounds__(256) k_sumsq(const double *__restrict__ x, i64 n, int slot, double *__restrict__ partials) {
    double v = 0.0;
    for (i64 i = (i64)blockIdx.x * 256 + threadIdx.x; i < n; i += (i64)gridDim.x * 256) v += x[i] * x[i];
    __shared__ double red[4];
#pragma unroll
    for (int off = 32; off >= 1; off >>= 1) v += __shfl_down(v, off, 64);
    if ((threadIdx.x & 63) == 0) red[threadIdx.x >> 6] = v;
    __syncthreads();
    if (threadIdx.x < S_COUNT)
        partials[(i64)blockIdx.x * S_COUNT + threadIdx.x] = ((int)threadIdx.x == slot) ? ((red[0] + red[1]) + red[2]) + red[3] : 0.0;
}

#define BND_TC 8
template <bool WEIGHTED, int DIR, bool NOMOM = false>
__global__ void __launch_bounds__(256) k_kkt_bnd(Grid g, LoopCoef c, KktCoef k, FusedGeom fg, const double *__restrict__ q,
                                                  const double *__restrict__ alpha, const double *__restrict__ weight,
                                                  const double *__restrict__ q2, const double *__restrict__ sx,
                                                  const double *__restrict__ sy, double *__restrict__ partials) {
    auto wgt = [&](i64 idx) { return WEIGHTED ? weight[idx] : 1.0; };
    auto rhoT_at = [&](i64 yy, i64 xx, i64 tl) -> double {
        if (tl < 0 || tl >= g.ncl) return 0.0;
        const i64 cidx = yy + g.py * (xx + g.nx * tl);
        return k.kappa * (wgt(cidx) * alpha[cidx]);
    };
    auto rho_node = [&](i64 yy, i64 xx, i64 tl) { return (rhoT_at(yy, xx, tl - 1) + rhoT_at(yy, xx, tl)) / 2.0; };
    double sM = 0.0, sR = 0.0, sF = 0.0, sD = 0.0;
    const i64 u = (i64)blockIdx.x * 256 + threadIdx.x;
    const i64 tbeg = (i64)blockIdx.z * BND_TC, tend = (tbeg + BND_TC < g.ntl) ? tbeg + BND_TC : g.ntl;
    for (i64 tl = tbeg; tl < tend; ++tl) {
    if (tl == 0 && !g.first) continue;
    if (DIR == 0) {
        const i64 y = u, x = (i64)blockIdx.y * TILE_X + (TILE_X - 1);
        if (y < g.ny && x < g.nx - 1) {
            const i64 e = g.offBx + g.bxLayer * tl + y + g.py * x;
            if (!NOMOM) {
                const double rm = (rho_node(y, x, tl) + rho_node(y, x + 1, tl)) / 2.0;
                const double rb = k.dsD * (rm * q[e]);
                const double m = k.kappa * (wgt(e) * alpha[e]);
                const double d = m - rb;
                sM += d * d;
                sR += rb * rb;
            }
            const double gb = c.sf * (q2[e] + sx[(tl * fg.nxblk + (x / TILE_X + 1)) * g.ny + y]);
            sF += gb * gb;
            const double r2 = gb + wgt(e) * alpha[e];
            sD += r2 * r2;
        }
    } else {
        const i64 x = u, y = (i64)blockIdx.y * 64 + 63;
        if (x < g.nx && y < g.ny - 1) {
            const i64 e = g.offBy + g.byLayer * tl + y + g.pyb * x;
            if (!NOMOM) {
                const double rm = (rho_node(y, x, tl) + rho_node(y + 1, x, tl)) / 2.0;
                const double rb = k.dsD * (rm * q[e]);
                const double m = k.kappa * (wgt(e) * alpha[e]);
                const double d = m - rb;
                sM += d * d;
                sR += rb * rb;
            }
            const double gb = c.sf * (q2[e] + sy[(tl * g.nx + x) * fg.nyblk + (y / 64 + 1)]);
            sF += gb * gb;
            const double r2 = gb + wgt(e) * alpha[e];
            sD += r2 * r2;
        }
    }
    }
    __shared__ double red[4][4];
    double v4[4] = {sM, sR, sF, sD};
    const int lane = threadIdx.x & 63, wv = threadIdx.x >> 6;
#pragma unroll
    for (int i = 0; i < 4; ++i) {
        double v = v4[i];
#pragma unroll
        for (int off = 32; off >= 1; off >>= 1) v += __shfl_down(v, off, 64);
        if (lane == 0) red[wv][i] = v;
    }
    __syncthreads();
    if (threadIdx.x < S_COUNT) {
        const int s = threadIdx.x;
        const int i = (s == S_MRHOB) ? 0 : (s == S_RHOB2) ? 1 : (s == S_FBBETA2) ? 2 : (s == S_DUAL2) ? 3 : -1;
        double v = 0.0;
        if (i >= 0) v = ((red[0][i] + red[1][i]) + red[2][i]) + red[3][i];
        const i64 bb = blockIdx.x + (i64)gridDim.x * (blockIdx.y + (i64)gridDim.y * blockIdx.z);
        partials[bb * S_COUNT + s] = v;
    }
}

__global__ void __launch_bounds__(256) k_kkt_final(const double *__restrict__ partials, i64 nblocks,
                                                    double *__restrict__ sums) {
    const int s = blockIdx.x;
    const i64 per = (nblocks + gridDim.y - 1) / gridDim.y;
    const i64 b0 = (i64)blockIdx.y * per, b1 = (b0 + per < nblocks) ? b0 + per : nblocks;
    double v = 0.0;
    for (i64 b = b0 + threadIdx.x; b < b1; b += 256) v += partials[b * S_COUNT + s];
    __shared__ double red[256];
    red[threadIdx.x] = v;
    __syncthreads();
    for (int off = 128; off >= 1; off >>= 1) {
        if ((int)threadIdx.x < off) red[threadIdx.x] += red[threadIdx.x + off];
        __syncthreads();
    }
    if (threadIdx.x == 0) sums[(i64)blockIdx.y * S_COUNT + s] = red[0];
}

__global__ void __launch_bounds__(64) k_kkt_final2(const double *__restrict__ slices, int nslices, double *__restrict__ sums) {
    const int s = threadIdx.x;
    if (s >= S_COUNT) return;
    double v = 0.0;
    for (int j = 0; j < nslices; ++j) v += slices[(i64)j * S_COUNT + s];
    sums[s] = v;
}

static void kkt_geometry(const Grid &g, dim3 &grid, i64 &chunk) {
    const i64 tiles = ((g.ny + TILE_Y - 1) / TILE_Y) * ((g.nx + TILE_X - 1) / TILE_X);
    i64 chunks = (4096 + tiles - 1) / tiles;
    if (chunks < 1) chunks = 1;
    if (chunks > g.ntl) chunks = g.ntl;
    chunk = (g.ntl + chunks - 1) / chunks;
    chunks = (g.ntl + chunk - 1) / chunk;
    grid = dim3((unsigned)((g.ny + TILE_Y - 1) / TILE_Y), (unsigned)((g.nx + TILE_X - 1) / TILE_X), (unsigned)chunks);
}

static i64 bnd_blocks(const Grid &g, const FusedGeom &fg, int dir) {
    const i64 tch = (g.ntl + BND_TC - 1) / BND_TC;
    if (dir == 0) return ((g.ny + 255) / 256) * fg.nxblk * tch;
    return ((g.nx + 255) / 256) * fg.nyblk * tch;
}

static i64 kkt_region_blocks(const Grid &g) {
    dim3 grid;
    i64 chunk;
    kkt_geometry(g, grid, chunk);
    FusedGeom fg;
    fused_geometry(g, fg);
    i64 m = (i64)grid.x * grid.y * grid.z;
    const i64 cand[] = {fg.nyblk * fg.nxblk * fg.chunks, qstep_rhs_blocks(g, fg), bnd_blocks(g, fg, 0), bnd_blocks(g, fg, 1)};
    for (i64 v : cand) m = v > m ? v : m;
    return m;
}

#define KKT_REGIONS 8
i64 kkt_partials_needed(const Grid &g) { return KKT_REGIONS * kkt_region_blocks(g); }

int launch_kkt(const Grid &g, const LoopCoef &c, const KktCoef &k, const double *phi, const double *q,
               const double *alpha, const double *z, const double *beta, const double *cvec, const double *weight,
               const KktHalo &halo, const KktWork &w, int parts, hipStream_t st, bool layer0, double *resid) {
    dim3 grid;
    i64 chunk;
    kkt_geometry(g, grid, chunk);
    const i64 region = kkt_region_blocks(g);
    if (KKT_REGIONS * region > w.maxBlocks) {
        set_error("kkt workspace too small");
        return DOTSOCP_EINVAL;
    }
    const int base = layer0 ? 4 : 0;
    if (layer0) { chunk = 1; grid.z = 1; }
    const dim3 blk(TILE_Y, TILE_X);
#define KKT_PART(W, P, slot)                                                                                     \
    if (parts & P)                                                                                               \
    DS_KLAUNCH((k_kkt<W, P>), grid, blk, 0, st, g, c, k, chunk, phi, q, alpha, z, beta, cvec, weight, halo, \
                       w.partials + ((layer0 && (slot) > 0 ? (slot) - 1 : (slot)) + base) * region * S_COUNT,    \
                       (P == 1) ? resid : nullptr)
    if (weight) { KKT_PART(true, 1, 0); KKT_PART(true, 2, 1); KKT_PART(true, 4, 2); KKT_PART(true, 8, 3); }
    else { KKT_PART(false, 1, 0); KKT_PART(false, 2, 1); KKT_PART(false, 4, 2); KKT_PART(false, 8, 3); }
#undef KKT_PART
    DS_HIP(hipGetLastError());
    return 0;
}

int launch_kkt_nodual(const Grid &g, const LoopCoef &c, const KktCoef &k, const double *phi, const double *q,
                      const double *alpha, const double *cvec, const double *weight, const KktWork &w, hipStream_t st) {
    dim3 grid;
    i64 chunk;
    kkt_geometry(g, grid, chunk);
    const i64 region = kkt_region_blocks(g);
    if (KKT_REGIONS * region > w.maxBlocks) {
        set_error("kkt workspace too small");
        return DOTSOCP_EINVAL;
    }
    const dim3 blk(TILE_Y, TILE_X);
    const KktHalo halo{nullptr, nullptr, nullptr, nullptr};
    const double *none = nullptr;
#define KKT_ND(W, P, reg)                                                                                                 \
    DS_KLAUNCH((k_kkt<W, P, true>), grid, blk, 0, st, g, c, k, chunk, phi, q, alpha, none, none, cvec, weight, halo, \
               w.partials + (i64)(reg) * region * S_COUNT, (double *)nullptr)
    if (weight) { KKT_ND(true, 1, 0); KKT_ND(true, 16, 4); KKT_ND(true, 4, 5); KKT_ND(true, 8, 6); }
    else { KKT_ND(false, 1, 0); KKT_ND(false, 16, 4); KKT_ND(false, 4, 5); KKT_ND(false, 8, 6); }
#undef KKT_ND
    DS_HIP(hipGetLastError());
    return 0;
}

int launch_kkt_bnd_dual(const Grid &g, const LoopCoef &c, const KktCoef &k, const FusedGeom &fg, const double *q,
                        const double *alpha, const double *weight, const double *q2, const double *sx, const double *sy,
                        const KktWork &w, hipStream_t st) {
    const i64 region = kkt_region_blocks(g);
    for (int dir = 0; dir < 2; ++dir) {
        const i64 len = dir == 0 ? g.ny : g.nx, lines = dir == 0 ? fg.nxblk : fg.nyblk;
        if (len <= 0 || lines <= 0) continue;
        dim3 gb((unsigned)((len + 255) / 256), (unsigned)lines, (unsigned)((g.ntl + BND_TC - 1) / BND_TC));
        double *pb = w.partials + (2 + dir) * region * S_COUNT;
#define BND(W, D) DS_KLAUNCH((k_kkt_bnd<W, D, true>), gb, dim3(256), 0, st, g, c, k, fg, q, alpha, weight, q2, sx, sy, pb)
        if (weight) { if (dir == 0) BND(true, 0); else BND(true, 1); }
        else { if (dir == 0) BND(false, 0); else BND(false, 1); }
#undef BND
        DS_HIP(hipGetLastError());
    }
    return 0;
}

int launch_kkt_cells_update(const Grid &g, const LoopCoef &c, const KktCoef &k, const FusedGeom &fg, FusedArgs a,
                            const double *phi, const double *alpha, const double *weight, const KktWork &w,
                            hipStream_t st, bool edges, const double *q_new) {
    if (g.Nz <= 0) return 0;
    const i64 region = kkt_region_blocks(g);
    a.TC = fg.TC;
    dim3 grid((unsigned)fg.nyblk, (unsigned)fg.nxblk, (unsigned)fg.chunks);
    double *part = w.partials + 1 * region * S_COUNT;
    const dim3 blk(TILE_Y, TILE_X);
    if (!edges) {
        if (weight) DS_KLAUNCH((k_kkt_cells<true, false>), grid, blk, 0, st, g, c, k, a, phi, alpha, weight, part);
        else DS_KLAUNCH((k_kkt_cells<false, false>), grid, blk, 0, st, g, c, k, a, phi, alpha, weight, part);
        DS_HIP(hipGetLastError());
        return 0;
    }
    const bool nt = stream_nt_enabled();
    if (weight) {
        if (nt) DS_KLAUNCH((k_kkt_cells<true, true, false, true>), grid, blk, 0, st, g, c, k, a, phi, alpha, weight, part);
        else DS_KLAUNCH((k_kkt_cells<true, true>), grid, blk, 0, st, g, c, k, a, phi, alpha, weight, part);
    } else {
        if (nt) DS_KLAUNCH((k_kkt_cells<false, true, false, true>), grid, blk, 0, st, g, c, k, a, phi, alpha, weight, part);
        else DS_KLAUNCH((k_kkt_cells<false, true>), grid, blk, 0, st, g, c, k, a, phi, alpha, weight, part);
    }
    DS_HIP(hipGetLastError());
    for (int dir = 0; dir < 2; ++dir) {
        const i64 len = dir == 0 ? g.ny : g.nx, lines = dir == 0 ? fg.nxblk : fg.nyblk;
        if (len <= 0 || lines <= 0) continue;
        dim3 gb((unsigned)((len + 255) / 256), (unsigned)lines, (unsigned)((g.ntl + BND_TC - 1) / BND_TC));
        double *pb = w.partials + (2 + dir) * region * S_COUNT;
#define BND(W, D) DS_KLAUNCH((k_kkt_bnd<W, D>), gb, dim3(256), 0, st, g, c, k, fg, q_new, alpha, weight, a.q2, a.sx, a.sy, pb)
        if (weight) { if (dir == 0) BND(true, 0); else BND(true, 1); }
        else { if (dir == 0) BND(false, 0); else BND(false, 1); }
#undef BND
        DS_HIP(hipGetLastError());
    }
    return 0;
}

int launch_norms(const Grid &g, const LoopCoef &c, const KktCoef &k, const FusedGeom &fg, FusedArgs a, const double *phi,
                 const double *alpha, const double *weight, const KktWork &w, hipStream_t st) {
    const i64 region = kkt_region_blocks(g);
    a.TC = fg.TC;
    if (g.Nz > 0) {
        dim3 grid((unsigned)fg.nyblk, (unsigned)fg.nxblk, (unsigned)fg.chunks);
        double *part = w.partials + 1 * region * S_COUNT;
        if (weight) DS_KLAUNCH((k_kkt_cells<true, false, true>), grid, dim3(TILE_Y, TILE_X), 0, st, g, c, k, a, phi, alpha, weight, part);
        else DS_KLAUNCH((k_kkt_cells<false, false, true>), grid, dim3(TILE_Y, TILE_X), 0, st, g, c, k, a, phi, alpha, weight, part);
    }
    struct R { const double *x; i64 n; int slot, reg; };
    const R rs[] = {{phi, g.Nphi, S_PHI2, 0},
                    {a.q, g.Nz, S_Q2, 2}, {a.q + g.offBx, g.bxLayer * g.ntl, S_Q2, 3}, {a.q + g.offBy, g.byLayer * g.ntl, S_Q2, 4},
                    {alpha, g.Nz, S_ALPHA2, 5}, {alpha + g.offBx, g.bxLayer * g.ntl, S_ALPHA2, 6},
                    {alpha + g.offBy, g.byLayer * g.ntl, S_ALPHA2, 7}};
    for (const R &r : rs) {
        if (r.n <= 0) continue;
        i64 blocks = (r.n + 256 * 64 - 1) / (256 * 64);
        if (blocks > region) blocks = region;
        double *part = w.partials + r.reg * region * S_COUNT;
        DS_KLAUNCH(k_sumsq, dim3((unsigned)blocks), dim3(256), 0, st, r.x, r.n, r.slot, part);
    }
    DS_HIP(hipGetLastError());
    return 0;
}

double *kkt_qstep_partials(const Grid &g, const KktWork &w) {
    (void)g;
    return w.partials;
}

int launch_kkt_final(const Grid &g, const KktWork &w, hipStream_t st) {
    DS_KLAUNCH(k_kkt_final, dim3(S_COUNT, KKT_SLICES), dim3(256), 0, st, w.partials,
                       KKT_REGIONS * kkt_region_blocks(g), w.sums + S_COUNT);
    DS_KLAUNCH(k_kkt_final2, dim3(1), dim3(64), 0, st, w.sums + S_COUNT, KKT_SLICES, w.sums);
    DS_HIP(hipGetLastError());
    return 0;
}

}
```

dot-socp_amd/csrc/solver.h:

```cpp
#pragma once
#include <chrono>
#include <functional>
#include <memory>
#include <string>
#include <vector>

#include "hostmem.h"
#include "kernels.h"

namespace dotsocp {

int guarded_malloc(void **p, size_t bytes);
void guarded_free(void *p);
long long device_cache_release();
int canary_check(std::string *report);
bool canary_enabled();
bool stream_stress_enabled();
void stream_stress(hipStream_t st);

template <class T>
inline int dmalloc(T **p, i64 n) {
    *p = nullptr;
    if (n <= 0) n = 1;
    return guarded_malloc((void **)p, sizeof(T) * (size_t)n);
}

inline void dfree(void *p) {
    if (p) guarded_free(p);
}

struct DevRes {
    int dev = 0;
    DctPlan *py = nullptr, *px = nullptr, *pt = nullptr;
    double *cy = nullptr, *cx = nullptr, *ct = nullptr;
};

#define DS_XEV 8
enum SlabEvent { EV_FORK = 0, EV_JOIN, EV_HALO, EV_CJOIN, EV_TRI, EV_MSG, EV_GOT, EV_X0 };
struct Slab {
    int index = 0;
    int dev = 0;
    hipStream_t st = nullptr;
    hipStream_t st_z = nullptr;
    hipEvent_t ev[EV_X0 + DS_XEV] = {nullptr};
    int xev_next = 0;
    DevRes *res = nullptr;
    double *h_sums = nullptr;
    Grid g;
    std::vector<void *> owned;
    template <class T> int alloc(T **p, i64 n) {
        DS_CHECK(dmalloc(p, n));
        owned.push_back(*p);
        return 0;
    }
    int zalloc(double **p, i64 n) {
        DS_CHECK(alloc(p, n));
        DS_HIP(hipMemsetAsync(*p, 0, sizeof(double) * (size_t)(n > 0 ? n : 1), st));
        return 0;
    }
    double *phi = nullptr;
    double *q = nullptr;
    double *alpha = nullptr;
    double *z = nullptr;
    double *beta = nullptr;
    double *c = nullptr;
    bool c_ends = false;
    double *weight = nullptr;
    double *w0 = nullptr, *w1 = nullptr;
    i64 l0 = 0, nl = 0;
    double *pencil = nullptr, *pencil2 = nullptr;
    double *stage = nullptr;
    double *u0_prev = nullptr, *tail_bx = nullptr, *tail_by = nullptr;
    double *a0_prev = nullptr, *a0w_prev = nullptr, *btail_bx = nullptr, *btail_by = nullptr;
    double *send_plane = nullptr, *send_plane2 = nullptr, *send_bx = nullptr, *send_by = nullptr;
    KktWork kw{};
    double *q_old = nullptr, *q2 = nullptr, *beta2 = nullptr, *sx = nullptr, *sy = nullptr;
    double *q3 = nullptr, *p2 = nullptr, *sxp = nullptr, *syp = nullptr;
    double *send_pbx = nullptr, *send_pby = nullptr, *ptail_bx = nullptr, *ptail_by = nullptr;
    double *alpha2 = nullptr;
    double *sx2 = nullptr, *sy2 = nullptr;
    double *tri_send = nullptr, *tri_recv = nullptr, *tri_bsend = nullptr, *tri_brecv = nullptr, *tri_zero = nullptr;
    double *carry = nullptr;
    FusedGeom fg{};
    double *phi_p = nullptr, *alpha_p = nullptr, *z_p = nullptr;
    double *phi_a = nullptr, *q_a = nullptr, *alpha_a = nullptr, *z_a = nullptr, *beta_a = nullptr;
    double *rep_edges = nullptr, *rep_part = nullptr, *rep_sums = nullptr;
    unsigned long long *rep_counts = nullptr;
    double *adv_vel = nullptr;
    i64 adv_have[2] = {-1, -1};
};

#define FOR_SLABS(s) for (auto &s : slabs) if (int rc_use__ = use(s)) return rc_use__; else

int dotsocp_slab_range_impl(i64 nt, int world, int rank, i64 *t0, i64 *t1);
void pencil_range(i64 plane, int world, int j, i64 *l0, i64 *l1);

bool if_adjust_sigma(double iter, double last_iter);

enum Phase { PH_RHS = 0, PH_POISSON, PH_PROJ, PH_QSTEP, PH_BETA, PH_KKT, PH_FUSED_A, PH_FUSED_B, PH_MATERIALISE,
             PH_COMM, PH_INTERP, PH_ACC_CONE, PH_ACC_GATHER, PH_QSTEP0, PH_TRANSPOSE, PH_CONE_CARRY, PH_QCONE, PH_VELOCITY, PH_ADVECT,
             PH_DEPOSIT, PH_FRAME_L1, PH_ADVECT_PATH, PH_MAP_FINAL, PH_COUNT };

bool rescale_due(i64 it, int rescale, double maxFeas, double relGap);
bool cone_writes_beta(i64 it, double lastSigmaIt, i64 maxit, bool checkStepByStep, bool last_of_run, int rescale,
                      double maxFeas, double relGap);

enum { QCONE_NONE = 0, QCONE_STEADY = 1, QCONE_EXIT = 2 };
int qcone_form(i64 it, double lastSigmaIt, i64 maxit, bool checkStepByStep, bool last_of_run, bool next_last_of_run,
               int rescale, double maxFeas, double relGap);

struct Solver {
    dotsocp_problem prob{};
    int device = 0;
    i64 ny = 0, nx = 0, nt = 0;
    hipStream_t stream = nullptr;
    hipStream_t stream_z = nullptr;
    bool multi_device = false;
    int ndev_visible = 1;
    std::vector<DevRes *> devres;
    int cur_dev = -1;
    std::vector<Slab> slabs;
    std::unique_ptr<DeferCtx> defer;
    int world = 1;
    int rank = 0;
    void *nccl = nullptr;
    double *h_sums = nullptr;
    double *d_red = nullptr;
    bool fused = true;
    bool overlap = false;
    bool tri_tsolve = true;
    bool peer_ok = true;
    bool cross_device = false;
    ~Solver();
    int init(const dotsocp_problem *p, int device, int nslabs, bool multi_dev = false);
    int attach_rccl(const unsigned char *id, int rank, int world);
    int use(const Slab &s);
    int use_dev(int d);
    int sync_all();
    DevRes *res_for(int dev);
    i64 column_pad() const;
    i64 row_pitch() const;
    int alloc_slabs(int first, int count);
    int ensure_alloc();
    void free_slabs();
    bool multi() const { return world > 1; }
    bool remote() const { return nccl != nullptr; }

    int xcopy(Slab &from, const double *src, Slab &to, double *dst, i64 count);
    int xcopy2d(Slab &from, const double *src, size_t spitch, Slab &to, double *dst, size_t dpitch, size_t width,
                size_t height);
    bool comm_z = false;
    bool comm_async = false;
    int comm_depth = 0;
    hipStream_t cst(const Slab &s) const { return comm_z ? s.st_z : s.st; }
    int comm_enter();
    int comm_leave();
    int comm_fork();
    int comm_mark(SlabEvent ev);
    int comm_wait(SlabEvent ev);
    int open_groups = 0;
    typedef std::function<double *(Slab &)> Sel;
    int shift(int dir, const Sel &src, const Sel &dst, i64 count);
    int shift_edge_halo(const Sel &base);
    int group_begin();
    int group_end();
    struct Msg { int from, to; const double *src; double *dst; i64 count; };
    std::vector<Msg> msgs;
    int msg_depth = 0;
    bool pull_default(const char *env_var) const;
    bool msg_batching() const;
    int flush_msgs();
    bool halo_pending = false;
    bool u0_fresh = false;
    bool u0_made = false;
    int make_u0_tail();
    int exchange_u0_tail();
    int exchange_q_halo(bool with_u0);
    int ensure_halo();
    int make_tails();
    int send_tails();
    int send_phi_head();
    int ship_tails();
    int transpose(bool forward);
    struct PhiHooks { std::function<int()> fill, behind; };
    int tri_alloc();
    int tri_exchange(bool back);
    int poisson_t_tridiag(const PhiHooks *hooks);

    i64 field_len(int field) const;
    enum { ROWS_DOWN = 0, ROWS_UP = 1, ROWS_FROM_DEV = 2 };
    int copy_rows(double *dev, double *host, i64 rowlen, i64 pitch, i64 nrows, int dir, hipStream_t st, int src_dev = -1);
    int upload(int field, const double *host);
    int upload_layers(int field, const double *host, i64 t0, i64 n);
    int download(int field, double *host);
    int upload_weight_from(const double *src, int src_dev, i64 src_ny, i64 src_nx, i64 src_nt);
    bool c_ends_on = true;
    int detect_c_ends();
    int stage_left_tail();
    int stage_rho_ends(Slab &s, const double *rho0, const double *rho1);
    int canary_after();
    int recover_outputs(const double *rho0, const double *rho1, double *rho, double *Ex, double *Ey, double *q0,
                        double *bx, double *by);
    int jump_from(Solver &coarse);
    int solution_report(const double *rho0, const double *rho1, dotsocp_report *rep, double *layer_mass, double *layer_neg);
    int render_evolution(const double *rho0, const double *rho1, const dotsocp_render_opts *o, const i64 *frame_nodes,
                         const double *levels, const unsigned char *lut, const unsigned char *barrier, unsigned char *image,
                         double *mvX, double *mvY, dotsocp_render_info *info);

    int velocity_stage(const double *rho0, const double *rho1);
    int velocity_layer(Slab &s, i64 tg, double floor);
    int recover_velocity(const double *rho0, const double *rho1, double floor, double *vX, double *vY);
    int advect_particles(const double *rho0, const double *rho1, const dotsocp_advect_opts *o, double *x, double *y,
                         double *traj_x, double *traj_y, i64 *n_clamped);
    int push_mass(const double *rho0, const double *rho1, const dotsocp_push_opts *o, double *x, double *y, const double *mass,
                  const i64 *frame_nodes, double *frames, i64 *n_clamped, double *unit, double *l1);
    int map_report(const double *rho0, const double *rho1, const dotsocp_advect_opts *o, double *x, double *y, const double *mass,
                   dotsocp_map_report_t *rep, double *disp, double *len, double *action);

    bool begun = false, finished = false, stopped = false;
    dotsocp_opts opts{};
    bool checkPrimDualFeas = true;
    double time_limit = 3600.0;
    double sigma = 1.0, sigmaScale = 1.0;
    double cScale = 1.0, dScale = 1.0, D = 1.0, E = 1.0;
    double norm_c = 0.0, norm_d = 0.0;
    double h = 1.0;
    int rescale = 0, use_feasOrg = 0;
    double maxFeas = 0.0, relGap = 0.0, tol_feasOrg = 0.0;
    double lastSigmaIt = 0.0;
    i64 it = 0;
    LoopCoef lc{};
    std::vector<double> hist_kkt, hist_time, hist_iter, hist_gap;
    std::chrono::steady_clock::time_point t_begin;
    double elapsed_prev = 0.0;
    double elapsed_agreed = 0.0;
    bool deferred = false;
    bool z_valid = true;
    bool z_prev_ok = false;
    bool rhs_valid = false;
    bool cone_carry = true;
    bool beta_gamma = false;
    bool cone_gout = false;
    bool last_of_run = false;
    int qcone = -1;
    bool q_valid = true;
    bool early_pass = false;
    bool early_gout = false;
    bool next_last_of_run = false;
    int need_q(const char *who) const;
    int qcone_decide() const;
    bool time_limit_passed() const;
    i64 timeout_at = -1;
    bool timeout_pending = false;
    int need_beta_form(const char *who) const;
    ScaleOps bops{0, 1.0, 1.0, 1.0, 1.0};
    ScaleOps zp_ops{0, 1.0, 1.0, 1.0, 1.0};
    int push_beta_op(double mul, double div);
    int flush_beta();
    ScaleOps aops{0, 1.0, 1.0, 1.0, 1.0};
    int flush_alpha();
    int sigma_scale_folded(double factor);
    FusedArgs pending_step_args(const Slab &s) const;
    double last_S[S_COUNT] = {0};
    double last_S_sigma = 1.0;
    i64 last_S_it = -1;
    bool norm_cache = true;
    bool kkt_fold = true;
    KktCoef kkt_coef() const;
    int clear_partials(Slab &s);
    int begin(const dotsocp_opts *o);
    int begin_method(const dotsocp_opts *o, int method, const dotsocp_acc_opts *acc);
    int run(i64 n_iters, i64 *done);
    int finish(dotsocp_result *res);
    int step(bool *brk);
    int rescale_block();
    int poisson_all(const PhiHooks *hooks = nullptr);
    int poisson_phi();
    int phase_phi(const PhiHooks *hooks = nullptr);
    int phase_z(int part = 0);
    int phase_q(int part = 0, bool kkt = false, int early = QCONE_NONE);
    int phase_mult();
    int materialise();
    int ensure_z();
    int kkt_sums(double *S, bool folded = false);
    int reduce_sums(double *S);
    int norms_light(double *S);
    int kkt_block(bool adjustSigmaYes, bool timed_out, bool *brk, bool folded = false);
    int scale_state(double a_mul, double a_div, double q_div, bool with_c);
    void update_coef();
    double elapsed() const;
    bool profiling = false;
    struct Pending { hipEvent_t a, b; int phase; };
    std::vector<Pending> pending;
    std::vector<hipEvent_t> event_pool;
    double phase_ms[PH_COUNT] = {0};
    i64 phase_launches[PH_COUNT] = {0};
    void prof_begin(int phase, bool on_z = false);
    void prof_end(int phase, bool on_z = false);
    int prof_flush();

    int method = DOTSOCP_METHOD_INPALM;
    i64 acc_restart = 100, acc_k = 0;
    double acc_rho = 2.0, acc_theta = 2.0;
    bool acc_halpern = true;
    bool acc_gather_valid = false;
    bool acc_swapped = false;
    bool acc_post = true;
    bool acc_light = false;
    double acc_factor = 1.0;
    int acc_alloc();
    int acc_begin(const dotsocp_acc_opts *acc);
    int acc_step(bool *brk);
    int acc_rescale_block();
    int acc_set_anchors();
    void acc_swap_state();
    int acc_on_sigma_factor(double factor);
    AccCoef acc_coef() const;
    bool palm_fast = true;
    bool palm_p_valid = false;
    int palm_begin();
    int palm_step(bool *brk);
};

struct DeviceScratch {
    Solver &S;
    std::vector<double *> bufs;
    explicit DeviceScratch(Solver &s) : S(s) {}
    int alloc(double **p, i64 n) { DS_CHECK(dmalloc(p, n)); bufs.push_back(*p); return 0; }
    ~DeviceScratch() {
        if (bufs.empty()) return;
        S.cur_dev = -1;
        (void)S.sync_all();
        for (double *b : bufs) dfree(b);
    }
};

}
```

dot-socp_amd/csrc/solver.hip:

```cpp
#include "solver.h"

#include <algorithm>
#include <cmath>
#include <cstring>

#include "comm.h"

namespace dotsocp {

void Solver::update_coef() {
    lc.s = E / D;
    lc.sf = edge_factor(lc.s);
    lc.dF = E / dScale;
    const double ht = 1.0 / (double)(nt - 1);
    lc.at = D * (1.0 / ht);
    lc.ax = (nx > 1) ? D * (1.0 / (1.0 / (double)(nx - 1))) : 0.0;
    lc.ay = (ny > 1) ? D * (1.0 / (1.0 / (double)(ny - 1))) : 0.0;
    lc.tau = opts.tau;
    const double tmp = (E / D) * (E / D);
    if (prob.weighted) { lc.c1 = 2.0 * tmp; lc.c2 = tmp; }
    else { lc.c1 = 1.0 + 2.0 * tmp; lc.c2 = 1.0 + tmp; }
    lc.dinv1 = 1.0 / lc.c1;
    lc.dinv2 = 1.0 / lc.c2;
}

int Solver::need_beta_form(const char *who) const {
    if (!beta_gamma) return 0;
    set_error("internal: %s met the gamma form of beta", who);
    return DOTSOCP_ESTATE;
}

int Solver::need_q(const char *who) const {
    if (q_valid) return 0;
    set_error("internal: %s met a q that was never stored", who);
    return DOTSOCP_ESTATE;
}

int Solver::flush_beta() {
    DS_CHECK(need_beta_form("flush_beta"));
    if (bops.empty()) return 0;
    FOR_SLABS(s) {
        DS_CHECK(launch_scale(s.beta, 10 * s.g.Nc, bops.mul, bops.div, s.st));
        if (bops.n > 1) DS_CHECK(launch_scale(s.beta, 10 * s.g.Nc, bops.mul2, bops.div2, s.st));
    }
    bops.clear();
    return 0;
}

int Solver::push_beta_op(double mul, double div) {
    if (bops.push(mul, div)) return 0;
    DS_CHECK(flush_beta());
    bops.push(mul, div);
    return 0;
}

FusedArgs Solver::pending_step_args(const Slab &s) const {
    FusedArgs a{};
    a.q_old = s.q_old;
    a.q = s.q;
    a.beta_in = s.beta;
    a.bops = bops;
    return a;
}

int Solver::clear_partials(Slab &s) {
    DS_HIP(ds_memset_async(s.kw.partials, 0, sizeof(double) * s.kw.maxBlocks * S_COUNT, s.st));
    return 0;
}

int Solver::flush_alpha() {
    if (aops.empty()) return 0;
    FOR_SLABS(s) DS_CHECK(launch_scale(s.alpha, s.g.NqAlloc, aops.mul, aops.div, s.st));
    aops.clear();
    return 0;
}

int Solver::sigma_scale_folded(double factor) {
    DS_CHECK(flush_alpha());
    DS_CHECK(ensure_halo());
    u0_made = false;
    DS_CHECK(push_beta_op(1.0, factor));
    if (multi()) {
        FOR_SLABS(s) DS_CHECK(launch_scale(s.alpha, s.g.NqAlloc, 1.0, factor, s.st));
    } else {
        aops.push(1.0, factor);
    }
    u0_fresh = false;
    FOR_SLABS(s) DS_CHECK(launch_rhs_sigma_fix(s.g, s.w0, s.w1, s.c, factor, s.st, c_ends_on && s.c_ends));
    return 0;
}

int Solver::scale_state(double a_mul, double a_div, double q_div, bool with_c) {
    DS_CHECK(need_beta_form("scale_state"));
    DS_CHECK(need_q("scale_state"));
    DS_CHECK(flush_alpha());
    if (begun) DS_CHECK(ensure_halo());
    u0_made = false;
    u0_fresh = false;
    rhs_valid = false;
    if (fused && begun) {
        DS_CHECK(push_beta_op(a_mul, a_div));
    }
    FOR_SLABS(s) {
        const Grid &g = s.g;
        if (with_c) DS_CHECK(launch_scale(s.c, g.Nphi, a_mul, a_div, s.st));
        if (!acc_light) DS_CHECK(launch_scale(s.alpha, g.NqAlloc, a_mul, a_div, s.st));
        if (!(fused && begun) && !acc_light) DS_CHECK(launch_scale(s.beta, 10 * g.Nc, a_mul, a_div, s.st));
        if (q_div != 1.0) {
            DS_CHECK(launch_scale(s.q, g.NqAlloc, 1.0, q_div, s.st));
            if (!(fused && begun) || z_valid) DS_CHECK(launch_scale(s.z, 10 * g.Nc, 1.0, q_div, s.st));
        }
    }
    if (q_div != 1.0 && fused && begun && !z_valid) z_prev_ok = false;
    return 0;
}

int Solver::begin_method(const dotsocp_opts *o, int m, const dotsocp_acc_opts *acc) {
    if (begun) { set_error("begin() called twice"); return DOTSOCP_ESTATE; }
    if (m == DOTSOCP_METHOD_INPALM) return begin(o);
    DS_ARG(m == DOTSOCP_METHOD_ACCADMM || m == DOTSOCP_METHOD_PALM, "unknown method");
    DS_ARG(prob.dim == 2, "the reference has PALM and acc-ADMM loops for 2-D problems only");
    DS_ARG(!(m == DOTSOCP_METHOD_PALM && prob.weighted), "the reference has no weighted PALM loop");
    method = m;
    int rc = begin(o);
    if (rc != 0) { method = DOTSOCP_METHOD_INPALM; return rc; }
    return (m == DOTSOCP_METHOD_PALM) ? palm_begin() : acc_begin(acc);
}

int Solver::begin(const dotsocp_opts *o) {
    DS_ARG(o != nullptr, "opts is NULL");
    DS_ARG(o->maxit >= 0, "opts.maxit < 0");
    DS_ARG(o->sigma > 0, "opts.sigma must be positive");
    if (begun) { set_error("begin() called twice"); return DOTSOCP_ESTATE; }
    cur_dev = -1;
    DS_CHECK(use_dev(device));
    DS_CHECK(ensure_alloc());
    if (method == DOTSOCP_METHOD_ACCADMM) {
        DS_CHECK(acc_alloc());
        fused = false;
    }
    opts = *o;
    cone_carry = true;
    if (const char *e = getenv("DOTSOCP_CONE_CARRY")) cone_carry = (atoi(e) != 0);
    c_ends_on = true;
    if (const char *e = getenv("DOTSOCP_C_ENDS")) c_ends_on = (atoi(e) != 0);
    if (c_ends_on) DS_CHECK(detect_c_ends());
    timeout_at = -1;
    if (const char *e = getenv("DOTSOCP_TEST_TIMEOUT_AT")) timeout_at = atoll(e);
    qcone = -1;
    if (const char *e = getenv("DOTSOCP_QCONE")) qcone = atoi(e);
    if (qcone < -1 || qcone > 2) qcone = -1;
    q_valid = true;
    early_pass = false;
    early_gout = false;
    next_last_of_run = false;
    beta_gamma = false;
    cone_gout = false;
    last_of_run = false;
    timeout_pending = false;
    checkPrimDualFeas = (o->checkPrimDualFeas < 0) ? !prob.weighted : (o->checkPrimDualFeas != 0);
    time_limit = (o->time_limit > 0) ? o->time_limit : 3600.0;
    sigma = o->sigma;
    lastSigmaIt = -INFINITY;
    cScale = prob.cScale; dScale = prob.dScale; D = prob.D; E = prob.E;
    use_feasOrg = 0;
    tol_feasOrg = 5 * o->tol;
    rescale = o->scaling ? 1 : 0;
    maxFeas = INFINITY; relGap = INFINITY;
    h = 1.0 / ((double)nx * (double)ny * (double)nt);
    norm_c = prob.normc; norm_d = prob.normd;
    update_coef();
    DS_CHECK(scale_state(1.0, sigma, 1.0, true));
    DS_CHECK(exchange_q_halo(false));
    sigmaScale = 1.0;
    it = 0;
    stopped = false;
    deferred = false;
    z_valid = true;
    z_prev_ok = false;
    rhs_valid = false;
    last_S_it = -1;
    hist_kkt.clear(); hist_time.clear(); hist_iter.clear(); hist_gap.clear();
    for (int i = 0; i < PH_COUNT; ++i) { phase_ms[i] = 0; phase_launches[i] = 0; }
    if (canary_enabled() && getenv("DOTSOCP_CANARY_SELFTEST")) {
        Slab &s0 = slabs[0];
        DS_CHECK(use(s0));
        const double v = 1.0;
        DS_HIP(ds_memcpy_async(s0.c + s0.g.Nphi, &v, sizeof v, hipMemcpyHostToDevice, s0.st));
        DS_HIP(ds_stream_synchronize(s0.st));
    }
    begun = true;
    elapsed_prev = 0.0;
    elapsed_agreed = 0.0;
    t_begin = std::chrono::steady_clock::now();
    return 0;
}

int Solver::poisson_all(const PhiHooks *hooks) {
    const i64 plane = slabs[0].g.plane;
    const bool tp2 = dct_plan_has_tsolve(devres[0]->pt);
    FOR_SLABS(s) {
        const Grid &g = s.g;
        DS_CHECK(launch_dct_axis(s.res->py, s.w0, s.w1, g.ny, g.nx, g.ntl, 0, 0, s.st, g.py));
        DS_CHECK(launch_dct_axis(s.res->px, s.w1, s.w0, g.ny, g.nx, g.ntl, 1, 0, s.st, g.py));
    }
    bool tri = multi() && tri_tsolve && world <= DS_MAX_WORLD;
    for (auto &s : slabs) tri = tri && s.g.ntl <= TRI_EXTRA;
    if (tri) {
        DS_CHECK(poisson_t_tridiag(hooks));
    } else {
    if (hooks && hooks->fill) {
        prof_end(PH_POISSON);
        DS_CHECK(hooks->fill());
        prof_begin(PH_POISSON);
    }
    if (hooks && hooks->behind) DS_CHECK(hooks->behind());
    if (multi()) {
        prof_begin(PH_TRANSPOSE);
        DS_CHECK(transpose(true));
        prof_end(PH_TRANSPOSE);
    }
    FOR_SLABS(s) {
        double *p = multi() ? s.pencil : s.w0;
        double *p2 = multi() ? s.pencil2 : s.w1;
        if (!multi()) {
            DS_CHECK(launch_poisson_t_single(s.res->pt, s.g, D * D, s.res->cy, s.res->cx, s.res->ct, p, p2, s.g.py, s.st, tri_tsolve));
        } else if (tp2) {
            DS_CHECK(launch_dct_t_solve(s.res->pt, p, p, s.g.py, plane, s.l0, s.nl, nt, D * D, s.res->cy, s.res->cx, s.res->ct, s.st));
        } else {
            DS_CHECK(launch_dct_axis(s.res->pt, p, p2, s.nl, 1, nt, 2, 0, s.st));
            DS_CHECK(launch_spectral_divide_pencil(p2, s.g.py, s.l0, s.nl, nt, D * D, s.res->cy, s.res->cx, s.res->ct, s.st));
            DS_CHECK(launch_dct_axis(s.res->pt, p2, p, s.nl, 1, nt, 2, 1, s.st));
        }
    }
    if (multi()) {
        prof_begin(PH_TRANSPOSE);
        DS_CHECK(transpose(false));
        prof_end(PH_TRANSPOSE);
    }
    }
    FOR_SLABS(s) {
        const Grid &g = s.g;
        DS_CHECK(launch_dct_axis(s.res->px, s.w0, s.w1, g.ny, g.nx, g.ntl, 1, 1, s.st, g.py));
        DS_CHECK(launch_dct_axis(s.res->py, s.w1, s.phi, g.ny, g.nx, g.ntl, 0, 1, s.st, g.py));
    }
    return 0;
}

int Solver::poisson_phi() {
    if (begun) { set_error("poisson_phi() must precede begin()"); return DOTSOCP_ESTATE; }
    cur_dev = -1;
    DS_CHECK(use_dev(device));
    DS_CHECK(ensure_alloc());
    D = prob.D;
    FOR_SLABS(s) DS_HIP(ds_memcpy_async(s.w0, s.phi, sizeof(double) * (size_t)s.g.Nphi, hipMemcpyDeviceToDevice, s.st));
    DS_CHECK(poisson_all(nullptr));
    return sync_all();
}

int Solver::phase_phi(const PhiHooks *hooks) {
    DS_CHECK(ensure_halo());
    if (multi() && !u0_fresh) {
        DS_CHECK(make_u0_tail());
        prof_begin(PH_COMM, comm_z);
        DS_CHECK(exchange_u0_tail());
        prof_end(PH_COMM, comm_z);
    }
    prof_begin(PH_RHS);
    if (!rhs_valid) {
        DS_CHECK(need_q("phase_phi"));
        DS_CHECK(flush_alpha());
        FOR_SLABS(s) DS_CHECK(launch_rhs(s.g, lc, s.q, s.alpha, s.c, s.weight, s.u0_prev, s.w0, s.st, c_ends_on && s.c_ends));
    } else if (multi()) {
        FOR_SLABS(s)
            if (!s.g.first) DS_CHECK(launch_rhs_fixup(s.g, lc, s.u0_prev, s.w0, s.st));
    }
    rhs_valid = false;
    prof_end(PH_RHS);
    prof_begin(PH_POISSON);
    DS_CHECK(poisson_all(hooks));
    prof_end(PH_POISSON);
    return 0;
}

int Solver::phase_z(int part) {
    if (early_pass) {
        early_pass = false;
        if (part != 0 || !fused || !deferred || cone_gout != early_gout) {
            set_error("internal: the early cone pass wrote %s, the schedule asks for %s", early_gout ? "gamma" : "beta",
                      cone_gout ? "gamma" : "beta");
            return DOTSOCP_ESTATE;
        }
        return 0;
    }
    DS_CHECK(need_q("phase_z"));
    if (part != 1) DS_CHECK(ensure_halo());
    if (!fused) {
        prof_begin(PH_PROJ);
        FOR_SLABS(s) DS_CHECK(launch_cone_proj(s.g, lc, s.q, s.beta, s.z, s.st));
        prof_end(PH_PROJ);
        return 0;
    }
    const bool gin = beta_gamma, gout = deferred && cone_gout;
    if (gin && (!deferred || !bops.empty())) {
        set_error("internal: gamma form %s", deferred ? "with a pending scaling of beta" : "without a pending multiplier step");
        return DOTSOCP_ESTATE;
    }
    const int flavour = (gin ? CONE_GIN : 0) | (gout ? CONE_GOUT : 0);
    const int ph = deferred ? (gin ? PH_CONE_CARRY : PH_FUSED_B) : PH_FUSED_A;
    z_valid = false;
    z_prev_ok = false;
    prof_begin(ph);
    FOR_SLABS(s) {
        FusedArgs a{};
        a.q = s.q;
        a.q2 = s.q2;
        a.sx = s.sx;
        a.sy = s.sy;
        a.beta_in = s.beta;
        a.bops = bops;
        const i64 C = s.fg.chunks;
        const i64 z0 = (part == 2) ? C - 1 : 0;
        const i64 zc = (part == 0) ? C : ((part == 1) ? C - 1 : 1);
        if (deferred) {
            a.q_old = s.q_old;
            a.beta_out = s.beta2;
        }
        const int mode = deferred ? 1 : 0;
        if (s.carry && C > 1) {
            for (i64 z = z0; z < z0 + zc; ++z) {
                a.carry_in = (z > 0) ? s.carry : nullptr;
                a.carry_out = (z + 1 < C) ? s.carry : nullptr;
                DS_CHECK(launch_cone_fused(mode, s.g, lc, s.fg, a, s.st, z, 1, flavour));
            }
        } else {
            DS_CHECK(launch_cone_fused(mode, s.g, lc, s.fg, a, s.st, z0, zc, flavour));
        }
        if (deferred && part != 1) std::swap(s.beta, s.beta2);
    }
    prof_end(ph);
    if (part == 1) return 0;
    if (deferred) {
        bops.clear();
        beta_gamma = gout;
    }
    return 0;
}

KktCoef Solver::kkt_coef() const {
    KktCoef k;
    k.sigma = sigma;
    k.kappa = sigma * cScale * D;
    k.dsD = dScale / D;
    k.dsE = dScale / E;
    return k;
}

int Solver::phase_q(int part, bool kkt, int early) {
    if (!fused) DS_CHECK(flush_alpha());
    if (early != QCONE_NONE && (part != 0 || kkt || multi() || !fused || !deferred || !beta_gamma || !bops.empty())) {
        set_error("internal: early cone pass in a state it does not serve");
        return DOTSOCP_ESTATE;
    }
    const bool egout = (early == QCONE_STEADY);
    const int ph = (early != QCONE_NONE) ? PH_QCONE : PH_QSTEP;
    prof_begin(ph);
    FOR_SLABS(s) {
        hipStream_t st = s.st;
        if (early != QCONE_NONE && qcone != 2) {
            if (!s.sx2) {
                DS_CHECK(s.zalloc(&s.sx2, s.fg.sx_len));
                DS_CHECK(s.zalloc(&s.sy2, s.fg.sy_len));
            }
            QConeArgs a{};
            a.phi = s.phi; a.q2v = s.q2; a.sx = s.sx; a.sy = s.sy; a.cvec = s.c; a.alpha_in = s.alpha; a.gamma_in = s.beta;
            a.alpha_out = s.alpha2; a.rhs = s.w0; a.q_out = s.q_old; a.beta_out = s.beta2;
            a.q2_out = s.q; a.sx_out = s.sx2; a.sy_out = s.sy2;
            a.ap_on = aops.n; a.ap_mul = aops.mul; a.ap_div = aops.div;
            a.c_ends = (c_ends_on && s.c_ends) ? 1 : 0;
            DS_CHECK(launch_qcone(s.g, lc, s.fg, a, egout, st));
            std::swap(s.alpha, s.alpha2);
            std::swap(s.q, s.q_old);
            std::swap(s.q2, s.q_old);
            std::swap(s.sx, s.sx2);
            std::swap(s.sy, s.sy2);
            std::swap(s.beta, s.beta2);
        } else if (!fused) {
            DS_CHECK(launch_qstep(s.g, lc, s.phi, s.z, s.beta, s.weight, s.tail_bx, s.tail_by, s.q, s.alpha, s.st));
        } else {
            const i64 C = qstep_rhs_chunks(s.g, s.fg);
            i64 z0 = 0, zc = C, zs = 1;
            if (part == 1) { zc = C - 1; }
            else if (part == 2) { z0 = C - 1; zc = 1; }
            QStepExtra ex{};
            ex.aops = aops;
            ex.c_ends = (c_ends_on && s.c_ends) ? 1 : 0;
            if (multi() && !s.g.last && part != 1) ex.u0_tail = s.send_plane;
            if (kkt) {
                const KktCoef k = kkt_coef();
                ex.partials = kkt_qstep_partials(s.g, s.kw);
                ex.resid = s.w1;
                ex.kappa = k.kappa; ex.dsD = k.dsD;
            }
            DS_CHECK(launch_qstep_rhs(s.g, lc, s.fg, s.phi, s.q2, s.sx, s.sy, s.weight, s.tail_bx, s.tail_by, s.c,
                                      s.q_old, s.alpha, s.alpha2, s.w0, st, z0, zc, zs, &ex));
            if (part != 1) std::swap(s.alpha, s.alpha2);
            if (part != 1) std::swap(s.q, s.q_old);
            if (early != QCONE_NONE) {
                FusedArgs a{};
                a.q = s.q; a.q2 = s.q2; a.sx = s.sx; a.sy = s.sy;
                a.beta_in = s.beta; a.beta_out = s.beta2;
                a.bops = bops;
                DS_CHECK(launch_cone_fused(1, s.g, lc, s.fg, a, s.st, 0, s.fg.chunks, CONE_GIN | (egout ? CONE_GOUT : 0)));
                std::swap(s.beta, s.beta2);
            }
        }
    }
    prof_end(ph);
    if (part == 1) return 0;
    q_valid = true;
    if (early != QCONE_NONE) {
        q_valid = !egout || qcone == 2;
        beta_gamma = egout;
        z_valid = false;
        z_prev_ok = false;
        early_pass = true;
        early_gout = egout;
    }
    u0_made = multi() && fused;
    if (fused) aops.clear();
    rhs_valid = fused;
    if (multi() && fused && comm_z && cone_split_enabled()) halo_pending = true;
    else DS_CHECK(exchange_q_halo(true));
    return 0;
}

int Solver::phase_mult() {
    if (fused) {
        deferred = true;
        return 0;
    }
    prof_begin(PH_BETA);
    FOR_SLABS(s) DS_CHECK(launch_beta_update(s.g, lc, s.q, s.z, s.beta, s.st));
    prof_end(PH_BETA);
    return 0;
}

int Solver::materialise() {
    if (!fused || !deferred) return 0;
    DS_CHECK(need_beta_form("materialise"));
    DS_CHECK(need_q("materialise"));
    DS_CHECK(ensure_halo());
    prof_begin(PH_MATERIALISE);
    FOR_SLABS(s) {
        FusedArgs a = pending_step_args(s);
        a.beta_out = s.beta;
        a.z_out = s.z;
        DS_CHECK(launch_cone_fused(2, s.g, lc, s.fg, a, s.st));
    }
    prof_end(PH_MATERIALISE);
    bops.clear();
    deferred = false;
    z_valid = true;
    return 0;
}

int Solver::ensure_z() {
    if (!fused || z_valid) return 0;
    DS_CHECK(need_beta_form("ensure_z"));
    DS_CHECK(need_q("ensure_z"));
    if (deferred) return materialise();
    if (!z_prev_ok) {
        set_error("internal: z cannot be regenerated");
        return DOTSOCP_ESTATE;
    }
    DS_CHECK(ensure_halo());
    prof_begin(PH_MATERIALISE);
    FOR_SLABS(s) {
        FusedArgs a{};
        a.q_old = s.q_old;
        a.q = s.q;
        a.beta_in = s.beta2;
        a.z_out = s.z;
        a.bops = zp_ops;
        DS_CHECK(launch_cone_fused(3, s.g, lc, s.fg, a, s.st));
    }
    prof_end(PH_MATERIALISE);
    z_valid = true;
    return 0;
}

int Solver::kkt_sums(double *S, bool folded) {
    DS_CHECK(need_beta_form("kkt_sums"));
    DS_CHECK(need_q("kkt_sums"));
    DS_CHECK(ensure_halo());
    const KktCoef k = kkt_coef();
    if (method == DOTSOCP_METHOD_ACCADMM && folded) {
        FOR_SLABS(s) DS_CHECK(launch_kkt_nodual(s.g, lc, k, s.phi, s.q, s.alpha, s.c, s.weight, s.kw, s.st));
        return reduce_sums(S);
    }
    if (!folded) {
        DS_CHECK(flush_alpha());
        FOR_SLABS(s) DS_CHECK(clear_partials(s));
    }
    int rest = folded ? 0 : (1 | 4 | 8);
    if (fused && deferred) {
        FOR_SLABS(s) {
            FusedArgs a = pending_step_args(s);
            a.beta_out = s.beta2;
            if (folded) { a.q2 = s.q2; a.sx = s.sx; a.sy = s.sy; }
            DS_CHECK(launch_kkt_cells_update(s.g, lc, k, s.fg, a, s.phi, s.alpha, s.weight, s.kw, s.st, folded, s.q));
            std::swap(s.beta, s.beta2);
        }
        zp_ops = bops;
        bops.clear();
        deferred = false;
        z_valid = false;
        z_prev_ok = true;
    } else {
        if (folded) { set_error("internal: folded KKT sums without a pending multiplier step"); return DOTSOCP_ESTATE; }
        DS_CHECK(ensure_z());
        DS_CHECK(flush_beta());
        rest |= 2;
    }
    if (multi()) {
        const i64 plane = slabs[0].g.plane;
        u0_made = false;
        FOR_SLABS(s)
            if (!s.g.last)
                DS_CHECK(launch_kkt_tail(s.g, s.alpha, s.beta, s.weight, s.send_plane, s.send_plane2, s.send_bx, s.send_by,
                                         s.st));
        DS_CHECK(group_begin());
        DS_CHECK(shift(+1, [](Slab &s) { return s.send_plane; }, [](Slab &s) { return s.a0_prev; }, plane));
        DS_CHECK(shift(+1, [](Slab &s) { return s.send_plane2; }, [](Slab &s) { return s.a0w_prev; }, plane));
        DS_CHECK(shift(+1, [](Slab &s) { return s.send_bx; }, [](Slab &s) { return s.btail_bx; }, slabs[0].g.bxLayer));
        DS_CHECK(shift(+1, [](Slab &s) { return s.send_by; }, [](Slab &s) { return s.btail_by; }, slabs[0].g.byLayer));
        DS_CHECK(group_end());
    }
    FOR_SLABS(s) {
        KktHalo halo{s.a0_prev, s.a0w_prev, s.btail_bx, s.btail_by};
        if (rest) DS_CHECK(launch_kkt(s.g, lc, k, s.phi, s.q, s.alpha, s.z, s.beta, s.c, s.weight, halo, s.kw, rest, s.st));
        if (folded && !s.g.first)
            DS_CHECK(launch_kkt(s.g, lc, k, s.phi, s.q, s.alpha, s.z, s.beta, s.c, s.weight, halo, s.kw, 1 | 4 | 8, s.st, true,
                                s.w1));
    }
    return reduce_sums(S);
}

int Solver::reduce_sums(double *S) {
    for (int i = 0; i <= S_COUNT; ++i) S[i] = 0.0;
    FOR_SLABS(s) {
        DS_CHECK(launch_kkt_final(s.g, s.kw, s.st));
        if (remote()) break;
        DS_HIP(ds_memcpy_async(s.h_sums, s.kw.sums, sizeof(double) * S_COUNT, hipMemcpyDeviceToHost, s.st));
    }
    if (!remote()) {
        FOR_SLABS(s) {
            DS_HIP(ds_stream_synchronize(s.st));
            for (int i = 0; i < S_COUNT; ++i) S[i] += s.h_sums[i];
        }
    }
    S[S_COUNT] = elapsed();
    if (remote()) {
        Rccl &api = rccl_api();
        Slab &s = slabs[0];
        DS_CHECK(comm_enter());
        const hipStream_t cs = cst(s);
        DS_NCCL(api.AllReduce(s.kw.sums, d_red, S_COUNT, ncclDouble, ncclSum, (ncclComm_t)nccl, cs));
        h_sums[S_COUNT] = S[S_COUNT];
        DS_HIP(ds_memcpy_async(d_red + S_COUNT, h_sums + S_COUNT, sizeof(double), hipMemcpyHostToDevice, cs));
        DS_NCCL(api.AllReduce(d_red + S_COUNT, d_red + S_COUNT, 1, ncclDouble, ncclMax, (ncclComm_t)nccl, cs));
        DS_HIP(ds_memcpy_async(h_sums, d_red, sizeof(double) * (S_COUNT + 1), hipMemcpyDeviceToHost, cs));
        DS_CHECK(comm_leave());
        DS_HIP(ds_stream_synchronize(stream));
        for (int i = 0; i <= S_COUNT; ++i) S[i] = h_sums[i];
    }
    elapsed_agreed = S[S_COUNT];
    return 0;
}

int Solver::norms_light(double *S) {
    DS_CHECK(need_beta_form("norms_light"));
    DS_CHECK(need_q("norms_light"));
    DS_CHECK(ensure_halo());
    DS_CHECK(flush_alpha());
    const KktCoef k = kkt_coef();
    FOR_SLABS(s) {
        DS_CHECK(clear_partials(s));
        const FusedArgs a = pending_step_args(s);
        DS_CHECK(launch_norms(s.g, lc, k, s.fg, a, s.phi, s.alpha, s.weight, s.kw, s.st));
    }
    return reduce_sums(S);
}

int Solver::rescale_block() {
    bool scaleYes = false;
    double normPhis = 0, normAlps = 0;
    auto norms = [&](double &nPhis, double &nAlps) -> int {
        double S[S_COUNT + 1];
        double sig = sigma;
        if (method == DOTSOCP_METHOD_INPALM && fused && last_S_it == it - 1 && norm_cache) {
            for (int i = 0; i < S_COUNT; ++i) S[i] = last_S[i];
            sig = last_S_sigma;
        } else if (method == DOTSOCP_METHOD_INPALM && fused && deferred && norm_cache) {
            DS_CHECK(norms_light(S));
        } else {
            DS_CHECK(materialise());
            DS_CHECK(ensure_z());
            DS_CHECK(kkt_sums(S));
        }
        const double sh = sqrt(h);
        const double normPhi = sh * sqrt(S[S_PHI2]), normQ = sh * sqrt(S[S_Q2]), normZ = sh * sqrt(S[S_Z2]);
        const double normAlpha = sig * (sh * sqrt(S[S_ALPHA2])), normBeta = sig * (sh * sqrt(S[S_BETA2]));
        nPhis = std::max(std::max(normPhi, normQ), normZ);
        nAlps = std::max(normAlpha, normBeta);
        return 0;
    };
    if (rescale_due(it, rescale, maxFeas, relGap)) DS_CHECK(need_beta_form("rescale_block"));
    if (rescale >= 3 && (it % 100) == 0) {
        DS_CHECK(norms(normPhis, normAlps));
        const double ratio = std::max(normAlps, normPhis) / std::min(normAlps, normPhis);
        if (ratio > 1.2) scaleYes = true;
    }
    const bool first = (rescale == 1) && (maxFeas < 2e-2) && (it >= 10) && (relGap < 5e-2);
    const bool second = (rescale == 2) && (maxFeas < 5e-3) && (it >= 50) && (relGap < 1e-2);
    if (!(first || second || scaleYes)) return 0;
    if (!scaleYes) DS_CHECK(norms(normPhis, normAlps));
    DS_CHECK(materialise());
    const double dScale2 = normPhis, cScale2 = normAlps;
    sigma = sigma * (cScale2 / dScale2);
    norm_c = norm_c / cScale2;
    if (!prob.weighted) norm_d = norm_d / dScale2;
    DS_CHECK(scale_state(dScale2, cScale2 * cScale2, dScale2, true));
    if (method == DOTSOCP_METHOD_PALM) {
        FOR_SLABS(s) DS_CHECK(launch_scale(s.phi, s.g.NphiAlloc, 1.0, dScale2, s.st));
    }
    dScale = dScale2 * dScale;
    cScale = cScale2 * cScale;
    sigmaScale = sigmaScale * (cScale2 / dScale2);
    update_coef();
    rescale += 1;
    return 0;
}

bool rescale_due(i64 it, int rescale, double maxFeas, double relGap) {
    if (rescale >= 3 && (it % 100) == 0) return true;
    if (rescale == 1 && maxFeas < 2e-2 && it >= 10 && relGap < 5e-2) return true;
    if (rescale == 2 && maxFeas < 5e-3 && it >= 50 && relGap < 1e-2) return true;
    return false;
}

bool cone_writes_beta(i64 it, double lastSigmaIt, i64 maxit, bool checkStepByStep, bool last_of_run, int rescale,
                      double maxFeas, double relGap) {
    if (checkStepByStep || if_adjust_sigma((double)it, lastSigmaIt) || it >= maxit) return true;
    if (last_of_run) return true;
    return rescale_due(it + 1, rescale, maxFeas, relGap);
}

int qcone_form(i64 it, double lastSigmaIt, i64 maxit, bool checkStepByStep, bool last_of_run, bool next_last_of_run,
               int rescale, double maxFeas, double relGap) {
    if (cone_writes_beta(it, lastSigmaIt, maxit, checkStepByStep, last_of_run, rescale, maxFeas, relGap)) return QCONE_NONE;
    return cone_writes_beta(it + 1, lastSigmaIt, maxit, checkStepByStep, next_last_of_run, rescale, maxFeas, relGap)
               ? QCONE_EXIT : QCONE_STEADY;
}

bool Solver::time_limit_passed() const {
    return timeout_pending || (remote() ? false : (elapsed() > time_limit || (timeout_at > 0 && it >= timeout_at)));
}

int Solver::qcone_decide() const {
    if (qcone == 0 || !fused || multi() || prob.weighted || method != DOTSOCP_METHOD_INPALM) return QCONE_NONE;
    if (!deferred || !beta_gamma || !bops.empty()) return QCONE_NONE;
    const Slab &s = slabs[0];
    if (s.g.ncl < 1 || s.fg.XB != 4) return QCONE_NONE;
    if (qcone < 0 && s.fg.nyblk * s.fg.nxblk < 2048) return QCONE_NONE;
    if (time_limit_passed()) return QCONE_NONE;
    return qcone_form(it, lastSigmaIt, opts.maxit, opts.ifCheckStepByStep != 0, last_of_run, next_last_of_run, rescale,
                      maxFeas, relGap);
}

bool if_adjust_sigma(double iter, double last_iter) {
    const double passed = iter - last_iter;
    if (iter < 20 && passed >= 3) return true;
    if (iter < 50 && passed >= 6) return true;
    if (iter < 100 && passed >= 10) return true;
    if (iter < 200 && passed >= 15) return true;
    if (iter < 500 && passed >= 25) return true;
    return passed >= 40;
}

static const double kUpdateRule[11][2] = {
    {1.1, 1.10}, {1.2, 1.15}, {1.5, 1.20}, {2, 1.26}, {2.5, 1.28}, {3.33, 1.32},
    {5, 1.35}, {10, 1.40}, {20, 1.60}, {40, 1.80}, {50, 2.00}};

static double get_factor(double xi) {
    double factor = 1.0;
    for (int i = 0; i < 11; ++i) {
        if (xi >= kUpdateRule[i][0]) factor = kUpdateRule[i][1];
        else break;
    }
    return factor;
}

static void adjust_lagrangian_param(double &sigma, double xi, double &factor) {
    factor = 1.0;
    if (xi >= 1) factor = get_factor(xi);
    else if (xi < 1) factor = 1.0 / get_factor(1.0 / xi);
    if (factor != 1.0) {
        const double old = sigma;
        sigma = std::max(std::min(sigma * factor, 1e3), 1e-3);
        factor = sigma / old;
    }
}

int Solver::kkt_block(bool adjustSigmaYes, bool timed_out, bool *brk, bool folded) {
    double S[S_COUNT + 1];
    prof_begin(PH_KKT);
    DS_CHECK(kkt_sums(S, folded));
    prof_end(PH_KKT);
    if (remote()) timed_out = elapsed_agreed > time_limit;
    for (int i = 0; i < S_COUNT; ++i) last_S[i] = S[i];
    last_S_sigma = sigma;
    last_S_it = it;
    const double sh = sqrt(h);
    auto nrm = [&](int i) { return sh * sqrt(S[i]); };
    const double norm_q = nrm(S_Q2), norm_z = nrm(S_Z2), norm_Aphi = nrm(S_APHI2);
    const double norm_alpha = sigma * nrm(S_ALPHA2), norm_beta = sigma * nrm(S_BETA2);
    const double norm_FBbeta = sigma * nrm(S_FBBETA2);
    const double primFea1 = nrm(S_PRIM1), primFea2 = nrm(S_PRIM2);
    const double dualFea1 = sigma * nrm(S_DUAL1), dualFea2 = sigma * nrm(S_DUAL2);
    const double complem = nrm(S_COMPLEM);
    const double dotcomplem = nrm(S_DOTCOMP), normRho = nrm(S_RHO2), norm_rhoFq = nrm(S_RHOFQ2);
    const double mRhoB = nrm(S_MRHOB), normM = nrm(S_M2), normRhoB = nrm(S_RHOB2);
    const double kc = 1.0;
    const double den2 = prob.weighted ? (norm_q + norm_z) : norm_d;
    double org[7], res[5];
    org[0] = primFea1 / (kc * D / dScale + norm_Aphi + norm_q);
    org[1] = primFea2 / (kc * E / dScale + den2);
    org[2] = dualFea1 / (kc / cScale + norm_c);
    org[3] = complem / (kc * E / dScale + norm_z + norm_beta);
    org[4] = dualFea2 / (kc / cScale / D + norm_FBbeta + norm_alpha);
    org[5] = dotcomplem / (kc + normRho + norm_rhoFq);
    org[6] = mRhoB / (kc + normM + normRhoB);
    res[0] = primFea1 / (kc + norm_Aphi + norm_q);
    res[1] = primFea2 / (kc + den2);
    res[2] = dualFea1 / (kc + norm_c);
    res[3] = complem / (kc + norm_z + norm_beta);
    res[4] = dualFea2 / (kc + norm_FBbeta + norm_alpha);
    const double priVal = (sigma * cScale * dScale * h) * S[S_QALPHA];
    const double dualVal = (sigma * cScale * dScale * h) * S[S_CPHI];
    const double pdGap = fabs(priVal - dualVal) / (1 + fabs(priVal) + fabs(dualVal));
    for (int i = 0; i < 7; ++i) hist_kkt.push_back(org[i]);
    hist_time.push_back(remote() ? elapsed_agreed : elapsed());
    hist_iter.push_back((double)it);
    hist_gap.push_back(pdGap);
    double mstop = std::max(std::max(org[0], org[2]), org[5]);
    if (checkPrimDualFeas) mstop = std::max(mstop, org[6]);
    if (mstop < opts.tol || timed_out) {
        *brk = true;
        return 0;
    }
    const double maxRes = *std::max_element(res, res + 5);
    if (maxRes < tol_feasOrg) use_feasOrg = 1;
    if (adjustSigmaYes) {
        lastSigmaIt = (double)it;
        double resiPri, resiDual;
        if (use_feasOrg) { resiPri = std::max(org[0], org[1]); resiDual = std::max(org[2], org[4]); }
        else { resiPri = std::max(res[0], res[1]); resiDual = std::max(res[2], res[4]); }
        double factor;
        adjust_lagrangian_param(sigma, resiPri / resiDual, factor);
        if (factor != 1.0) {
            if (folded && rhs_valid && method != DOTSOCP_METHOD_ACCADMM) DS_CHECK(sigma_scale_folded(factor));
            else DS_CHECK(scale_state(1.0, factor, 1.0, true));
            if (method == DOTSOCP_METHOD_ACCADMM) DS_CHECK(acc_on_sigma_factor(factor));
        }
    }
    if (rescale > 0) {
        maxFeas = maxRes;
        relGap = pdGap;
    }
    return 0;
}

int Solver::step(bool *brk) {
    *brk = false;
    if (method == DOTSOCP_METHOD_ACCADMM) return acc_step(brk);
    if (method == DOTSOCP_METHOD_PALM) return palm_step(brk);
    it += 1;
    DS_CHECK(rescale_block());
    const bool adjustSigmaYes = if_adjust_sigma((double)it, lastSigmaIt);
    const bool early_steady = early_pass && early_gout;
    const bool kkt_due = opts.ifCheckStepByStep || adjustSigmaYes || it == opts.maxit || (timeout_pending && !early_steady);
    cone_gout = cone_carry && fused && deferred && !kkt_due &&
                !cone_writes_beta(it, lastSigmaIt, opts.maxit, opts.ifCheckStepByStep != 0, last_of_run, rescale, maxFeas, relGap);
    const bool fold = kkt_due && kkt_fold && fused;
    const bool inter = comm_z && multi() && fused;
    bool split = inter && cone_split_enabled();
    for (auto &s : slabs) split = split && s.fg.chunks >= 2;
    bool split_q = inter && cone_split_enabled();
    for (auto &s : slabs) split_q = split_q && qstep_rhs_chunks(s.g, s.fg) >= 2;
    auto async_comm = [&](const std::function<int()> &fn, SlabEvent ev) -> int {
        DS_CHECK(comm_fork());
        comm_async = true;
        const int rc = fn();
        comm_async = false;
        DS_CHECK(rc);
        return comm_mark(ev);
    };
    if (inter) {
        const bool pend = halo_pending;
        if (pend) {
            DS_CHECK(make_u0_tail());
            DS_CHECK(async_comm([&]() { return ensure_halo(); }, EV_HALO));
        }
        if (split) DS_CHECK(phase_z(1));
        if (pend) DS_CHECK(comm_wait(EV_HALO));
        if (!split) DS_CHECK(phase_z(0));
        PhiHooks hooks;
        hooks.fill = [&]() -> int {
            if (split) DS_CHECK(phase_z(2));
            return make_tails();
        };
        hooks.behind = [&]() -> int { return async_comm([&]() { return send_tails(); }, EV_JOIN); };
        DS_CHECK(phase_phi(&hooks));
    } else {
        DS_CHECK(phase_phi());
        DS_CHECK(phase_z(0));
    }
    if (fold) {
        FOR_SLABS(s) DS_CHECK(clear_partials(s));
    }
    if (inter) {
        DS_CHECK(async_comm([&]() { return send_phi_head(); }, EV_HALO));
        DS_CHECK(comm_wait(EV_JOIN));
        if (split_q) DS_CHECK(phase_q(1, fold));
        DS_CHECK(comm_wait(EV_HALO));
        DS_CHECK(phase_q(split_q ? 2 : 0, fold));
    } else {
        DS_CHECK(ship_tails());
        DS_CHECK(phase_q(0, fold, fold ? QCONE_NONE : qcone_decide()));
    }
    DS_CHECK(phase_mult());
    const bool timed_out = time_limit_passed();
    timeout_pending = false;
    if (timed_out && (beta_gamma || early_pass)) {
        timeout_pending = true;
        return 0;
    }
    if (kkt_due || timed_out)
        DS_CHECK(kkt_block(adjustSigmaYes, timed_out, brk, fold));
    return 0;
}

int Solver::run(i64 n_iters, i64 *done) {
    if (!begun || finished) { set_error("run() needs begin() and must precede finish()"); return DOTSOCP_ESTATE; }
    cur_dev = -1;
    DS_CHECK(use_dev(device));
    struct DeferScope {
        DeferCtx *ctx;
        int err = 0;
        explicit DeferScope(DeferCtx *c) : ctx(c) { if (ctx) { g_defer = ctx; ctx->begin(); } }
        int close() { if (ctx) { err = ctx->end(); g_defer = nullptr; ctx = nullptr; } return err; }
        ~DeferScope() { (void)close(); }
    } scope(defer.get());
    i64 n = 0;
    while (it < opts.maxit && !stopped) {
        if (n_iters >= 0 && n >= n_iters) break;
        bool brk = false;
        last_of_run = (n_iters >= 0 && n + 1 >= n_iters);
        next_last_of_run = (n_iters >= 0 && n + 2 >= n_iters);
        DS_CHECK(step(&brk));
        if (brk) stopped = true;
        ++n;
    }
    DS_CHECK(need_beta_form("the end of run()"));
    DS_CHECK(need_q("the end of run()"));
    if (early_pass) { set_error("internal: an early cone pass is pending at the end of run()"); return DOTSOCP_ESTATE; }
    DS_CHECK(ensure_halo());
    DS_CHECK(sync_all());
    DS_CHECK(prof_flush());
    if (const int derr = scope.close()) {
        set_error("a HIP call issued by a slab thread failed: %s", hipGetErrorString((hipError_t)derr));
        return DOTSOCP_EHIP;
    }
    if (done) *done = n;
    return 0;
}

int Solver::finish(dotsocp_result *res) {
    if (!begun) { set_error("finish() before begin()"); return DOTSOCP_ESTATE; }
    cur_dev = -1;
    DS_CHECK(use_dev(device));
    DS_CHECK(ensure_z());
    DS_CHECK(flush_beta());
    DS_CHECK(flush_alpha());
    DS_CHECK(sync_all());
    DS_CHECK(prof_flush());
    if (canary_enabled()) {
        std::string rep;
        const int bad = canary_check(&rep);
        cur_dev = -1;
        if (bad) {
            set_error("canary: %d device buffer(s) written out of bounds: %s", bad, rep.c_str());
            return DOTSOCP_EHIP;
        }
    }
    finished = true;
    if (res) {
        memset(res, 0, sizeof *res);
        res->sigma = sigma / sigmaScale;
        res->sigma_internal = sigma;
        res->cScale = cScale;
        res->dScale = dScale;
        res->times[0] = (phase_ms[PH_RHS] + phase_ms[PH_POISSON]) * 1e-3;
        res->times[1] = (phase_ms[PH_PROJ] + phase_ms[PH_FUSED_A] + phase_ms[PH_FUSED_B] + phase_ms[PH_CONE_CARRY]) * 1e-3;
        res->times[2] = phase_ms[PH_QSTEP] * 1e-3;
        res->times[3] = (phase_ms[PH_BETA] + phase_ms[PH_MATERIALISE]) * 1e-3;
        res->times[4] = phase_ms[PH_KKT] * 1e-3;
        res->times[5] = elapsed();
        res->times[6] = (double)it;
        res->iters = it;
        res->hist_len = (i64)hist_iter.size();
        res->stopped = stopped ? 1 : 0;
        if (method == DOTSOCP_METHOD_PALM) res->time_extra = phase_ms[PH_QSTEP0] * 1e-3;
        if (method == DOTSOCP_METHOD_ACCADMM) {
            res->times[0] = (phase_ms[PH_RHS] + phase_ms[PH_POISSON]) * 1e-3;
            res->times[1] = phase_ms[PH_ACC_CONE] * 1e-3;
            res->times[2] = (phase_ms[PH_QSTEP] + phase_ms[PH_ACC_GATHER]) * 1e-3;
            res->times[3] = 0.0;
            res->time_extra = phase_ms[PH_INTERP] * 1e-3;
        }
    }
    return 0;
}
void Solver::prof_begin(int phase, bool on_z) {
    if (!profiling) return;
    (void)use_dev(device);
    hipStream_t st = on_z ? stream_z : stream;
    Pending p;
    p.phase = phase;
    auto get = [&]() {
        hipEvent_t e;
        if (!event_pool.empty()) { e = event_pool.back(); event_pool.pop_back(); }
        else (void)hipEventCreate(&e);
        return e;
    };
    p.a = get();
    p.b = get();
    (void)ds_event_record(p.a, st);
    pending.push_back(p);
}

void Solver::prof_end(int phase, bool on_z) {
    if (!profiling) return;
    (void)use_dev(device);
    hipStream_t st = on_z ? stream_z : stream;
    for (auto it2 = pending.rbegin(); it2 != pending.rend(); ++it2)
        if (it2->phase == phase) { (void)ds_event_record(it2->b, st); break; }
}

int Solver::prof_flush() {
    if (!profiling || pending.empty()) return 0;
    DS_CHECK(use_dev(device));
    DS_HIP(ds_stream_synchronize(stream_z));
    DS_HIP(ds_stream_synchronize(stream));
    for (auto &p : pending) {
        float ms = 0.f;
        if (hipEventElapsedTime(&ms, p.a, p.b) == hipSuccess) {
            phase_ms[p.phase] += ms;
            phase_launches[p.phase] += 1;
        }
        event_pool.push_back(p.a);
        event_pool.push_back(p.b);
    }
    pending.clear();
    return 0;
}

double Solver::elapsed() const {
    return elapsed_prev + std::chrono::duration<double>(std::chrono::steady_clock::now() - t_begin).count();
}

}
```

include/dotsocp.h:

```cpp
#ifndef DOTSOCP_H
#define DOTSOCP_H

#ifdef __cplusplus
extern "C" {
#endif

typedef long long dotsocp_i64;

enum {
    DOTSOCP_OK = 0,
    DOTSOCP_EINVAL = -1,
    DOTSOCP_ENODEVICE = -2,
    DOTSOCP_EHIP = -3,
    DOTSOCP_ESTATE = -4,
    DOTSOCP_ECOMM = -5
};

const char *dotsocp_last_error(void);
const char *dotsocp_version(void);
int dotsocp_device_count(void);
dotsocp_i64 dotsocp_release_cache(void);


int dotsocp_proj_soc(double *out, const double *in, dotsocp_i64 M, dotsocp_i64 K);

int dotsocp_bfd(double *z, const double *q, dotsocp_i64 nt, dotsocp_i64 nx, dotsocp_i64 ny,
                double scale, double dF);

int dotsocp_bfd_conj(double *q, const double *z, dotsocp_i64 nt, dotsocp_i64 nx, dotsocp_i64 ny,
                     double scale);

int dotsocp_bfd1d(double *z, const double *q, dotsocp_i64 nt, dotsocp_i64 nx, double scale, double dF);

int dotsocp_bfd_conj1d(double *q, const double *z, dotsocp_i64 nt, dotsocp_i64 nx, double scale);

int dotsocp_oper_poisson(double *res, const double *rhs, dotsocp_i64 ny, dotsocp_i64 nx,
                         dotsocp_i64 nt, double kernelScale);

int dotsocp_dctn(double *a, dotsocp_i64 ny, dotsocp_i64 nx, dotsocp_i64 nt, int inverse);

int dotsocp_proj_soc_dev(double *d_out, const double *d_in, dotsocp_i64 M, dotsocp_i64 K, void *stream);
int dotsocp_bfd_dev(double *d_z, const double *d_q, dotsocp_i64 nt, dotsocp_i64 nx, dotsocp_i64 ny,
                    double scale, double dF, void *stream);
int dotsocp_bfd_conj_dev(double *d_q, const double *d_z, dotsocp_i64 nt, dotsocp_i64 nx, dotsocp_i64 ny,
                         double scale, void *stream);


typedef struct dotsocp_ctx dotsocp_ctx;

typedef struct {
    int dim;
    int weighted;
    dotsocp_i64 ny, nx, nt;
    double D, E;
    double cScale, dScale;
    double normc, normd;
} dotsocp_problem;

typedef struct {
    double tau;
    double sigma;
    double tol;
    dotsocp_i64 maxit;
    int ifCheckStepByStep;
    int checkPrimDualFeas;
    int scaling;
    double time_limit;
} dotsocp_opts;

enum {
    DOTSOCP_METHOD_INPALM = 0,
    DOTSOCP_METHOD_PALM = 1,
    DOTSOCP_METHOD_ACCADMM = 2
};

typedef struct {
    dotsocp_i64 restart;
    double rho;
    double theta;
} dotsocp_acc_opts;

enum {
    DOTSOCP_F_PHI = 0,
    DOTSOCP_F_Q = 1,
    DOTSOCP_F_ALPHA = 2,
    DOTSOCP_F_Z = 3,
    DOTSOCP_F_BETA = 4,
    DOTSOCP_F_C = 5,
    DOTSOCP_F_WEIGHT = 6
};

typedef struct {
    double sigma;
    double sigma_internal;
    double cScale, dScale;
    double times[7];
    dotsocp_i64 iters;
    dotsocp_i64 hist_len;
    int stopped;
    double time_extra;
} dotsocp_result;

dotsocp_ctx *dotsocp_create(const dotsocp_problem *prob, int device, int nslabs);
dotsocp_ctx *dotsocp_create_multi(const dotsocp_problem *prob, int first_device, int ngpu);
void dotsocp_destroy(dotsocp_ctx *ctx);

int dotsocp_rccl_unique_id(unsigned char id[128]);
int dotsocp_attach_rccl(dotsocp_ctx *ctx, const unsigned char id[128], int rank, int world);

int dotsocp_slab_range(dotsocp_i64 nt, int world, int rank, dotsocp_i64 *t0, dotsocp_i64 *t1);

dotsocp_i64 dotsocp_field_len(const dotsocp_problem *prob, int field);

int dotsocp_dct_algorithm(dotsocp_i64 n);

int dotsocp_cdft_levels(dotsocp_i64 n);

int dotsocp_dct_levels(dotsocp_i64 n, int axis);

int dotsocp_tsolve_tri_safe(dotsocp_i64 ny, dotsocp_i64 nx, dotsocp_i64 nt);

int dotsocp_cone_writes_beta(dotsocp_i64 it, double last_sigma_it, dotsocp_i64 maxit, int check_step_by_step,
                             int last_of_run, int rescale, double maxFeas, double relGap);
int dotsocp_rescale_due(dotsocp_i64 it, int rescale, double maxFeas, double relGap);
int dotsocp_qcone_form(dotsocp_i64 it, double last_sigma_it, dotsocp_i64 maxit, int check_step_by_step, int last_of_run,
                       int next_last_of_run, int rescale, double maxFeas, double relGap);

int dotsocp_upload(dotsocp_ctx *ctx, int field, const double *host);
int dotsocp_download(dotsocp_ctx *ctx, int field, double *host);
int dotsocp_upload_layers(dotsocp_ctx *ctx, int field, const double *host, dotsocp_i64 t0, dotsocp_i64 n);

int dotsocp_begin(dotsocp_ctx *ctx, const dotsocp_opts *opts);
int dotsocp_begin_method(dotsocp_ctx *ctx, const dotsocp_opts *opts, int method, const dotsocp_acc_opts *acc);
int dotsocp_run(dotsocp_ctx *ctx, dotsocp_i64 n_iters, dotsocp_i64 *done);
int dotsocp_finish(dotsocp_ctx *ctx, dotsocp_result *res);

int dotsocp_recover_outputs(dotsocp_ctx *ctx, const double *rho0, const double *rho1, double *rho, double *Ex,
                            double *Ey, double *q0, double *bx, double *by);

#define DOTSOCP_REPORT_BINS 49
#define DOTSOCP_REPORT_RHO_FLOOR 1e-8
typedef struct {
    dotsocp_i64 n_nodes, n_cells;
    double mass_err, neg_err;
    double rho_min;  dotsocp_i64 rho_neg;
    dotsocp_i64 rho_hist[DOTSOCP_REPORT_BINS];
    double fq_max;   dotsocp_i64 fq_pos;
    dotsocp_i64 fq_hist[DOTSOCP_REPORT_BINS];
    double cost;
    dotsocp_i64 nonfinite;
} dotsocp_report;

int dotsocp_report_edges(double edges[DOTSOCP_REPORT_BINS + 1]);
int dotsocp_solution_report(dotsocp_ctx *ctx, const double *rho0, const double *rho1, dotsocp_report *rep,
                            double *layer_mass , double *layer_neg );

int dotsocp_recover_velocity(dotsocp_ctx *ctx, const double *rho0, const double *rho1, double rho_floor,
                             double *vx, double *vy);

typedef struct { dotsocp_i64 n; int nsub; int direction; double rho_floor; } dotsocp_advect_opts;
int dotsocp_advect_particles(dotsocp_ctx *ctx, const double *rho0, const double *rho1, const dotsocp_advect_opts *o,
                             double *x, double *y, double *traj_x, double *traj_y, dotsocp_i64 *n_clamped);

typedef struct { dotsocp_i64 n; int nsub; int direction; double rho_floor; dotsocp_i64 nf; } dotsocp_push_opts;
int dotsocp_push_mass(dotsocp_ctx *ctx, const double *rho0, const double *rho1, const dotsocp_push_opts *o,
                      double *x, double *y, const double *mass, const dotsocp_i64 *frame_nodes, double *frames,
                      dotsocp_i64 *n_clamped, double *unit, double *l1);

typedef struct {
    dotsocp_i64 n, n_clamped, n_still;
    double mass;
    double cost_map, cost_length, cost_action;
    double disp_mean, len_mean;
    double disp_max, len_max, detour_max;
    dotsocp_i64 detour_hist[DOTSOCP_REPORT_BINS];
    dotsocp_i64 detour_over;
} dotsocp_map_report_t;
int dotsocp_map_report(dotsocp_ctx *ctx, const double *rho0, const double *rho1, const dotsocp_advect_opts *o,
                       double *x, double *y, const double *mass, dotsocp_map_report_t *rep, double *disp, double *len,
                       double *action);

enum { DOTSOCP_RENDER_LINEAR = 0, DOTSOCP_RENDER_INVERTED = 1, DOTSOCP_RENDER_LEVELS = 2 };
typedef struct {
    int mode;
    int channels;
    dotsocp_i64 nf;
    int nlevels;
    int barrier_index;
    double vmax;
    dotsocp_i64 skip_y, skip_x;
    double mask_frac;
} dotsocp_render_opts;
typedef struct {
    double vmax, rho_min;
    dotsocp_i64 nonfinite, masked;
    dotsocp_i64 my, mx;
} dotsocp_render_info;
int dotsocp_render_evolution(dotsocp_ctx *ctx, const double *rho0, const double *rho1, const dotsocp_render_opts *opts,
                             const dotsocp_i64 *frame_nodes, const double *levels, const unsigned char *lut,
                             const unsigned char *barrier, unsigned char *image, double *mvx, double *mvy,
                             dotsocp_render_info *info);

int dotsocp_jump_next_level(dotsocp_ctx *coarse, dotsocp_ctx *fine);

typedef struct dotsocp_weights dotsocp_weights;

dotsocp_weights *dotsocp_weights_create(int device, dotsocp_i64 ny, dotsocp_i64 nx, dotsocp_i64 nt, int levels);
void dotsocp_weights_destroy(dotsocp_weights *w);

dotsocp_i64 dotsocp_weights_len(dotsocp_i64 ny, dotsocp_i64 nx, dotsocp_i64 nt, int levels, int level);

int dotsocp_weights_set(dotsocp_weights *w, const double *weight);
int dotsocp_weights_set_space(dotsocp_weights *w, const double *weightX, const double *weightY);

int dotsocp_weights_restrict(dotsocp_weights *w, int log_mean);

int dotsocp_weights_log10_mean(dotsocp_weights *w, int level, double *mean);

int dotsocp_weights_download(dotsocp_weights *w, int level, double *host);

int dotsocp_upload_weight_from(dotsocp_ctx *ctx, dotsocp_weights *w, int level);

int dotsocp_get_history(dotsocp_ctx *ctx, double *kkt, double *time, double *iter, double *pdGap);

int dotsocp_set_profiling(dotsocp_ctx *ctx, int on);
int dotsocp_kernel_time(dotsocp_ctx *ctx, const char *name, double *avg_ms, dotsocp_i64 *launches);

int dotsocp_canary_check(void);

int dotsocp_poisson_phi(dotsocp_ctx *ctx);

int dotsocp_synchronize(dotsocp_ctx *ctx);

#ifdef __cplusplus
}
#endif
#endif
```

Baseline: 99.38.

## Keep multiplier step pending across folded KKT checks with sums-only cell pass

On folded KKT check iterations in the single-slab fused path, the KKT cell pass now computes residual sums without storing the updated beta, leaving the multiplier step deferred. Any sigma rescale from that check is carried as a pending scale op and applied inside the next cone pass (MODE_B or MODE_M), so beta is read and written once fewer per check. This adds state tracking, guard checks and new kernel template variants, and falls back to materialising beta on break, rescale or at the end of a run. Only single-GPU, unweighted INPALM runs with large grids qualify, so multi-GPU configurations see no change.

```diff
diff --git a/dot-socp_amd/capi.py b/dot-socp_amd/capi.py
--- a/dot-socp_amd/capi.py
+++ b/dot-socp_amd/capi.py
@@ -109,6 +109,7 @@
     "dotsocp_cone_writes_beta": (ctypes.c_int, [i64, dbl, i64, ctypes.c_int, ctypes.c_int, ctypes.c_int, dbl, dbl]),
     "dotsocp_rescale_due": (ctypes.c_int, [i64, ctypes.c_int, dbl, dbl]),
     "dotsocp_qcone_form": (ctypes.c_int, [i64, dbl, i64, ctypes.c_int, ctypes.c_int, ctypes.c_int, ctypes.c_int, dbl, dbl]),
+    "dotsocp_kkt_pend_form": (ctypes.c_int, [i64, i64, ctypes.c_int, ctypes.c_int, ctypes.c_int, ctypes.c_int, ctypes.c_int]),
     "dotsocp_release_cache": (i64, []),
     "dotsocp_upload": (ctypes.c_int, [vp, ctypes.c_int, vp]),
     "dotsocp_upload_layers": (ctypes.c_int, [vp, ctypes.c_int, vp, i64, i64]),
diff --git a/dot-socp_amd/csrc/capi.hip b/dot-socp_amd/csrc/capi.hip
--- a/dot-socp_amd/csrc/capi.hip
+++ b/dot-socp_amd/csrc/capi.hip
@@ -300,6 +300,10 @@
     return qcone_form(it, last_sigma_it, maxit, check_step_by_step != 0, last_of_run != 0, next_last_of_run != 0, rescale,
                       maxFeas, relGap);
 }
+int dotsocp_kkt_pend_form(dotsocp_i64 it, dotsocp_i64 maxit, int check_step_by_step, int last_of_run, int timed_out, int rescale,
+                          int eligible) {
+    return kkt_pend_form(it, maxit, check_step_by_step != 0, last_of_run != 0, timed_out != 0, rescale, eligible != 0) ? 1 : 0;
+}
 
 dotsocp_i64 dotsocp_field_len(const dotsocp_problem *p, int field) {
     if (!p || (p->dim != 1 && p->dim != 2) || p->nt < 2 || p->nx < 1 || (p->dim == 2 && p->ny < 1)) return -1;
diff --git a/dot-socp_amd/csrc/fused.hip b/dot-socp_amd/csrc/fused.hip
--- a/dot-socp_amd/csrc/fused.hip
+++ b/dot-socp_amd/csrc/fused.hip
@@ -6,9 +6,10 @@
 
 namespace dotsocp {
 
-template <int MODE, int XB, bool NT = false, bool GIN = false, bool GOUT = false>
+template <int MODE, int XB, bool NT = false, bool GIN = false, bool GOUT = false, bool POPS = false>
 __global__ void __launch_bounds__(64 * XB) k_cone_fused(Grid g, LoopCoef c, FusedArgs a) {
     static_assert(MODE == 1 || !(GIN || GOUT), "the gamma form exists between two MODE_B passes only");
+    static_assert(!POPS || ((MODE == 1 && !GIN) || MODE == 2), "a scaling behind the step: the beta-reading MODE_B passes and MODE_M");
     constexpr bool DUAL = (MODE >= 5);
     constexpr bool UPD = (MODE != 0 && MODE != 6);
     constexpr bool PROJ = (MODE < 2 || MODE >= 5);
@@ -66,6 +67,7 @@
                 proj_row<10>(zo);
 #pragma unroll
                 for (int j = 0; j < 10; ++j) b[j] = mult_finish(mult_carry(b[j], zo[j], c.tau), v[j], c.tau);
+                if constexpr (POPS) apply_scale_ops(b, a.pops);
                 if (own && inb) {
                     if (MODE != 3 && !GOUT) {
 #pragma unroll
@@ -181,6 +183,21 @@
         if (nt) DS_KLAUNCH((k_cone_fused<M, 4, true>), grid, blk, 0, st, g, c, a);       \
         else DS_KLAUNCH((k_cone_fused<M, 4>), grid, blk, 0, st, g, c, a);                \
         break;
+    if (!a.pops.empty()) {
+        if (!(mode == 1 && (flavour & ~CONE_GOUT) == 0) && !(mode == 2 && flavour == 0)) {
+            set_error("internal: a scaling behind the multiplier step in a pass that does not execute it");
+            return DOTSOCP_ESTATE;
+        }
+#define CONE_POPS(M, GO)                                                                              \
+        if (nt) DS_KLAUNCH((k_cone_fused<M, 4, true, false, GO, true>), grid, blk, 0, st, g, c, a);   \
+        else DS_KLAUNCH((k_cone_fused<M, 4, false, false, GO, true>), grid, blk, 0, st, g, c, a);
+        if (mode == 2) { CONE_POPS(2, false) }
+        else if (flavour == CONE_GOUT) { CONE_POPS(1, true) }
+        else { CONE_POPS(1, false) }
+#undef CONE_POPS
+        DS_HIP(hipGetLastError());
+        return 0;
+    }
     if (flavour != 0) {
         if (mode != 1 || (flavour & ~(CONE_GIN | CONE_GOUT))) { set_error("bad fused flavour"); return DOTSOCP_EINVAL; }
         if ((flavour & CONE_GIN) && !a.bops.empty()) { set_error("internal: gamma with a pending scaling"); return DOTSOCP_ESTATE; }
diff --git a/dot-socp_amd/csrc/kernels.h b/dot-socp_amd/csrc/kernels.h
--- a/dot-socp_amd/csrc/kernels.h
+++ b/dot-socp_amd/csrc/kernels.h
@@ -75,6 +75,7 @@
     int z0;
     const double *carry_in;
     double *carry_out;
+    ScaleOps pops;
 };
 bool tile_xcd_remap(const Grid &g);
 int fused_geometry(const Grid &g, FusedGeom &fg);
@@ -266,7 +267,7 @@
                         const KktWork &w, hipStream_t st);
 int launch_kkt_cells_update(const Grid &g, const LoopCoef &c, const KktCoef &k, const FusedGeom &fg, FusedArgs a,
                             const double *phi, const double *alpha, const double *weight, const KktWork &w,
-                            hipStream_t st, bool edges = false, const double *q_new = nullptr);
+                            hipStream_t st, bool edges = false, const double *q_new = nullptr, bool store = true);
 int launch_norms(const Grid &g, const LoopCoef &c, const KktCoef &k, const FusedGeom &fg, FusedArgs a, const double *phi,
                  const double *alpha, const double *weight, const KktWork &w, hipStream_t st);
 double *kkt_qstep_partials(const Grid &g, const KktWork &w);
diff --git a/dot-socp_amd/csrc/kkt.hip b/dot-socp_amd/csrc/kkt.hip
--- a/dot-socp_amd/csrc/kkt.hip
+++ b/dot-socp_amd/csrc/kkt.hip
@@ -178,8 +178,8 @@
     }
 }
 
-template <bool WEIGHTED, bool EDGES, bool NORMS = false, bool NT = false>
-__global__ void __launch_bounds__(TILE_Y *TILE_X) k_kkt_cells(Grid g, LoopCoef c, KktCoef k, FusedArgs a,
+template <bool WEIGHTED, bool EDGES, bool NORMS = false, bool NT = false, bool STORE = true>
+__global__ void __launch_bounds__(TILE_Y *TILE_X, STORE ? 1 : 3) k_kkt_cells(Grid g, LoopCoef c, KktCoef k, FusedArgs a,
                                                                const double *__restrict__ phi,
                                                                const double *__restrict__ alpha,
                                                                const double *__restrict__ weight,
@@ -224,6 +224,14 @@
                 for (int j = 0; j < 10; ++j) zo[j] = zo[j] - b[j];
                 proj_row<10>(zo);
                 double zs = 0.0, bs = 0.0, rs = 0.0;
+                double sq_early = 0.0;
+                if constexpr (!STORE) {
+#pragma unroll
+                    for (int j = 1; j < 9; ++j) {
+                        const double e = k.dsE * v[j];
+                        sq_early += e * e;
+                    }
+                }
 #pragma unroll
                 for (int j = 0; j < 10; ++j) {
                     const double r = zo[j] - v[j];
@@ -239,8 +247,10 @@
                     S[S_BETA2] += bs;
                 }
                 if (own && !NORMS) {
-#pragma unroll
-                    for (int j = 0; j < 10; ++j) st_stream<NT>(a.beta_out + j * g.Nc + i, b[j]);
+                    if constexpr (STORE) {
+#pragma unroll
+                        for (int j = 0; j < 10; ++j) st_stream<NT>(a.beta_out + j * g.Nc + i, b[j]);
+                    }
                     auto xj = [&](int j) { return zo[j] - k.sigma * b[j]; };
                     const double n = sqrt(soc_norm2(xj, 10)), x0 = xj(0);
                     double cf = (x0 / n + 1.0) * 0.5;
@@ -260,11 +270,13 @@
                     const double w = wgt(i);
                     const double av = alpha[i];
                     const double rhoT = k.kappa * (w * av);
-                    double sq = 0.0;
-#pragma unroll
-                    for (int j = 1; j < 9; ++j) {
-                        const double e = k.dsE * v[j];
-                        sq += e * e;
+                    double sq = sq_early;
+                    if constexpr (STORE) {
+#pragma unroll
+                        for (int j = 1; j < 9; ++j) {
+                            const double e = k.dsE * v[j];
+                            sq += e * e;
+                        }
                     }
                     double rhoFq = rhoT + k.dsD * q0 + sq / 4.0;
                     rhoFq = (rhoFq < 0.0) ? 0.0 : rhoFq;
@@ -572,8 +584,10 @@
 
 int launch_kkt_cells_update(const Grid &g, const LoopCoef &c, const KktCoef &k, const FusedGeom &fg, FusedArgs a,
                             const double *phi, const double *alpha, const double *weight, const KktWork &w,
-                            hipStream_t st, bool edges, const double *q_new) {
+                            hipStream_t st, bool edges, const double *q_new, bool store) {
     if (g.Nz <= 0) return 0;
+    if (!store && (!edges || weight)) { set_error("internal: the sums-only cell pass serves the folded check without a weight"); return DOTSOCP_ESTATE; }
+    if (!a.pops.empty()) { set_error("internal: the cell pass met a scaling behind the multiplier step"); return DOTSOCP_ESTATE; }
     const i64 region = kkt_region_blocks(g);
     a.TC = fg.TC;
     dim3 grid((unsigned)fg.nyblk, (unsigned)fg.nxblk, (unsigned)fg.chunks);
@@ -589,6 +603,9 @@
     if (weight) {
         if (nt) DS_KLAUNCH((k_kkt_cells<true, true, false, true>), grid, blk, 0, st, g, c, k, a, phi, alpha, weight, part);
         else DS_KLAUNCH((k_kkt_cells<true, true>), grid, blk, 0, st, g, c, k, a, phi, alpha, weight, part);
+    } else if (!store) {
+        if (nt) DS_KLAUNCH((k_kkt_cells<false, true, false, true, false>), grid, blk, 0, st, g, c, k, a, phi, alpha, weight, part);
+        else DS_KLAUNCH((k_kkt_cells<false, true, false, false, false>), grid, blk, 0, st, g, c, k, a, phi, alpha, weight, part);
     } else {
         if (nt) DS_KLAUNCH((k_kkt_cells<false, true, false, true>), grid, blk, 0, st, g, c, k, a, phi, alpha, weight, part);
         else DS_KLAUNCH((k_kkt_cells<false, true>), grid, blk, 0, st, g, c, k, a, phi, alpha, weight, part);
@@ -610,6 +627,7 @@
 
 int launch_norms(const Grid &g, const LoopCoef &c, const KktCoef &k, const FusedGeom &fg, FusedArgs a, const double *phi,
                  const double *alpha, const double *weight, const KktWork &w, hipStream_t st) {
+    if (!a.pops.empty()) { set_error("internal: the norms pass met a scaling behind the multiplier step"); return DOTSOCP_ESTATE; }
     const i64 region = kkt_region_blocks(g);
     a.TC = fg.TC;
     if (g.Nz > 0) {
diff --git a/dot-socp_amd/csrc/solver.h b/dot-socp_amd/csrc/solver.h
--- a/dot-socp_amd/csrc/solver.h
+++ b/dot-socp_amd/csrc/solver.h
@@ -109,6 +109,9 @@
 int qcone_form(i64 it, double lastSigmaIt, i64 maxit, bool checkStepByStep, bool last_of_run, bool next_last_of_run,
                int rescale, double maxFeas, double relGap);
 
+bool rescale_possible(i64 it, int rescale);
+bool kkt_pend_form(i64 it, i64 maxit, bool checkStepByStep, bool last_of_run, bool timed_out, int rescale, bool eligible);
+
 struct Solver {
     dotsocp_problem prob{};
     int device = 0;
@@ -259,7 +262,12 @@
     int flush_beta();
     ScaleOps aops{0, 1.0, 1.0, 1.0, 1.0};
     int flush_alpha();
-    int sigma_scale_folded(double factor);
+    int sigma_scale_folded(double factor, bool behind_step = false);
+    int kkt_pend = -1;
+    ScaleOps pops{0, 1.0, 1.0, 1.0, 1.0};
+    bool kkt_pend_eligible() const;
+    bool early_pass_eligible() const;
+    int settle_pops();
     FusedArgs pending_step_args(const Slab &s) const;
     double last_S[S_COUNT] = {0};
     double last_S_sigma = 1.0;
@@ -282,10 +290,10 @@
     int phase_mult();
     int materialise();
     int ensure_z();
-    int kkt_sums(double *S, bool folded = false);
+    int kkt_sums(double *S, bool folded = false, bool pend = false);
     int reduce_sums(double *S);
     int norms_light(double *S);
-    int kkt_block(bool adjustSigmaYes, bool timed_out, bool *brk, bool folded = false);
+    int kkt_block(bool adjustSigmaYes, bool timed_out, bool *brk, bool folded = false, bool pend = false);
     int scale_state(double a_mul, double a_div, double q_div, bool with_c);
     void update_coef();
     double elapsed() const;
diff --git a/dot-socp_amd/csrc/solver.hip b/dot-socp_amd/csrc/solver.hip
--- a/dot-socp_amd/csrc/solver.hip
+++ b/dot-socp_amd/csrc/solver.hip
@@ -36,8 +36,15 @@
     return DOTSOCP_ESTATE;
 }
 
+int Solver::settle_pops() {
+    if (pops.empty()) return 0;
+    if (!fused || !deferred) { set_error("internal: a scaling behind a multiplier step that is not pending"); return DOTSOCP_ESTATE; }
+    return materialise();
+}
+
 int Solver::flush_beta() {
     DS_CHECK(need_beta_form("flush_beta"));
+    DS_CHECK(settle_pops());
     if (bops.empty()) return 0;
     FOR_SLABS(s) {
         DS_CHECK(launch_scale(s.beta, 10 * s.g.Nc, bops.mul, bops.div, s.st));
@@ -60,6 +67,7 @@
     a.q = s.q;
     a.beta_in = s.beta;
     a.bops = bops;
+    a.pops = pops;
     return a;
 }
 
@@ -75,11 +83,18 @@
     return 0;
 }
 
-int Solver::sigma_scale_folded(double factor) {
+int Solver::sigma_scale_folded(double factor, bool behind_step) {
     DS_CHECK(flush_alpha());
     DS_CHECK(ensure_halo());
     u0_made = false;
-    DS_CHECK(push_beta_op(1.0, factor));
+    if (behind_step) {
+        if (!pops.push(1.0, factor) || pops.n != 1 || !deferred) {
+            set_error("internal: a second scaling behind the pending multiplier step");
+            return DOTSOCP_ESTATE;
+        }
+    } else {
+        DS_CHECK(push_beta_op(1.0, factor));
+    }
     if (multi()) {
         FOR_SLABS(s) DS_CHECK(launch_scale(s.alpha, s.g.NqAlloc, 1.0, factor, s.st));
     } else {
@@ -93,6 +108,7 @@
 int Solver::scale_state(double a_mul, double a_div, double q_div, bool with_c) {
     DS_CHECK(need_beta_form("scale_state"));
     DS_CHECK(need_q("scale_state"));
+    DS_CHECK(settle_pops());
     DS_CHECK(flush_alpha());
     if (begun) DS_CHECK(ensure_halo());
     u0_made = false;
@@ -150,6 +166,9 @@
     qcone = -1;
     if (const char *e = getenv("DOTSOCP_QCONE")) qcone = atoi(e);
     if (qcone < -1 || qcone > 2) qcone = -1;
+    kkt_pend = -1;
+    if (const char *e = getenv("DOTSOCP_KKT_PEND")) kkt_pend = (atoi(e) != 0) ? 1 : 0;
+    pops.clear();
     q_valid = true;
     early_pass = false;
     early_gout = false;
@@ -286,7 +305,7 @@
 int Solver::phase_z(int part) {
     if (early_pass) {
         early_pass = false;
-        if (part != 0 || !fused || !deferred || cone_gout != early_gout) {
+        if (part != 0 || !fused || !deferred || cone_gout != early_gout || !pops.empty()) {
             set_error("internal: the early cone pass wrote %s, the schedule asks for %s", early_gout ? "gamma" : "beta",
                       cone_gout ? "gamma" : "beta");
             return DOTSOCP_ESTATE;
@@ -304,6 +323,10 @@
     const bool gin = beta_gamma, gout = deferred && cone_gout;
     if (gin && (!deferred || !bops.empty())) {
         set_error("internal: gamma form %s", deferred ? "with a pending scaling of beta" : "without a pending multiplier step");
+        return DOTSOCP_ESTATE;
+    }
+    if (!pops.empty() && (!deferred || gin || part != 0)) {
+        set_error("internal: a scaling behind the multiplier step, and a cone pass that does not execute one");
         return DOTSOCP_ESTATE;
     }
     const int flavour = (gin ? CONE_GIN : 0) | (gout ? CONE_GOUT : 0);
@@ -325,6 +348,7 @@
         if (deferred) {
             a.q_old = s.q_old;
             a.beta_out = s.beta2;
+            a.pops = pops;
         }
         const int mode = deferred ? 1 : 0;
         if (s.carry && C > 1) {
@@ -342,6 +366,7 @@
     if (part == 1) return 0;
     if (deferred) {
         bops.clear();
+        pops.clear();
         beta_gamma = gout;
     }
     return 0;
@@ -358,7 +383,7 @@
 
 int Solver::phase_q(int part, bool kkt, int early) {
     if (!fused) DS_CHECK(flush_alpha());
-    if (early != QCONE_NONE && (part != 0 || kkt || multi() || !fused || !deferred || !beta_gamma || !bops.empty())) {
+    if (early != QCONE_NONE && (part != 0 || kkt || multi() || !fused || !deferred || !beta_gamma || !bops.empty() || !pops.empty())) {
         set_error("internal: early cone pass in a state it does not serve");
         return DOTSOCP_ESTATE;
     }
@@ -460,6 +485,7 @@
     }
     prof_end(PH_MATERIALISE);
     bops.clear();
+    pops.clear();
     deferred = false;
     z_valid = true;
     return 0;
@@ -490,7 +516,11 @@
     return 0;
 }
 
-int Solver::kkt_sums(double *S, bool folded) {
+int Solver::kkt_sums(double *S, bool folded, bool pend) {
+    if (pend && !(folded && fused && deferred && !multi())) {
+        set_error("internal: a pending check outside the folded single-slab path");
+        return DOTSOCP_ESTATE;
+    }
     DS_CHECK(need_beta_form("kkt_sums"));
     DS_CHECK(need_q("kkt_sums"));
     DS_CHECK(ensure_halo());
@@ -504,7 +534,15 @@
         FOR_SLABS(s) DS_CHECK(clear_partials(s));
     }
     int rest = folded ? 0 : (1 | 4 | 8);
-    if (fused && deferred) {
+    if (fused && deferred && pend) {
+        FOR_SLABS(s) {
+            FusedArgs a = pending_step_args(s);
+            a.q2 = s.q2; a.sx = s.sx; a.sy = s.sy;
+            DS_CHECK(launch_kkt_cells_update(s.g, lc, k, s.fg, a, s.phi, s.alpha, s.weight, s.kw, s.st, true, s.q, false));
+        }
+        z_valid = false;
+        z_prev_ok = false;
+    } else if (fused && deferred) {
         FOR_SLABS(s) {
             FusedArgs a = pending_step_args(s);
             a.beta_out = s.beta2;
@@ -668,12 +706,30 @@
     return timeout_pending || (remote() ? false : (elapsed() > time_limit || (timeout_at > 0 && it >= timeout_at)));
 }
 
+bool Solver::early_pass_eligible() const {
+    if (qcone == 0 || !fused || multi() || prob.weighted || method != DOTSOCP_METHOD_INPALM) return false;
+    const Slab &s = slabs[0];
+    if (s.g.ncl < 1 || s.fg.XB != 4) return false;
+    if (qcone < 0 && s.fg.nyblk * s.fg.nxblk < 2048) return false;
+    return true;
+}
+
+bool Solver::kkt_pend_eligible() const {
+    return kkt_pend != 0 && cone_carry && kkt_fold && early_pass_eligible();
+}
+
+bool rescale_possible(i64 it, int rescale) {
+    return rescale_due(it, rescale, 0.0, 0.0);
+}
+
+bool kkt_pend_form(i64 it, i64 maxit, bool checkStepByStep, bool last_of_run, bool timed_out, int rescale, bool eligible) {
+    if (!eligible || checkStepByStep || last_of_run || timed_out || it >= maxit) return false;
+    return !rescale_possible(it + 1, rescale);
+}
+
 int Solver::qcone_decide() const {
-    if (qcone == 0 || !fused || multi() || prob.weighted || method != DOTSOCP_METHOD_INPALM) return QCONE_NONE;
-    if (!deferred || !beta_gamma || !bops.empty()) return QCONE_NONE;
-    const Slab &s = slabs[0];
-    if (s.g.ncl < 1 || s.fg.XB != 4) return QCONE_NONE;
-    if (qcone < 0 && s.fg.nyblk * s.fg.nxblk < 2048) return QCONE_NONE;
+    if (!early_pass_eligible()) return QCONE_NONE;
+    if (!deferred || !beta_gamma || !bops.empty() || !pops.empty()) return QCONE_NONE;
     if (time_limit_passed()) return QCONE_NONE;
     return qcone_form(it, lastSigmaIt, opts.maxit, opts.ifCheckStepByStep != 0, last_of_run, next_last_of_run, rescale,
                       maxFeas, relGap);
@@ -713,10 +769,10 @@
     }
 }
 
-int Solver::kkt_block(bool adjustSigmaYes, bool timed_out, bool *brk, bool folded) {
+int Solver::kkt_block(bool adjustSigmaYes, bool timed_out, bool *brk, bool folded, bool pend) {
     double S[S_COUNT + 1];
     prof_begin(PH_KKT);
-    DS_CHECK(kkt_sums(S, folded));
+    DS_CHECK(kkt_sums(S, folded, pend));
     prof_end(PH_KKT);
     if (remote()) timed_out = elapsed_agreed > time_limit;
     for (int i = 0; i < S_COUNT; ++i) last_S[i] = S[i];
@@ -758,9 +814,14 @@
     if (checkPrimDualFeas) mstop = std::max(mstop, org[6]);
     if (mstop < opts.tol || timed_out) {
         *brk = true;
+        if (pend) DS_CHECK(materialise());
         return 0;
     }
     const double maxRes = *std::max_element(res, res + 5);
+    if (pend && rescale_due(it + 1, rescale, rescale > 0 ? maxRes : maxFeas, rescale > 0 ? pdGap : relGap)) {
+        set_error("internal: a pending check in front of a rescale block");
+        return DOTSOCP_ESTATE;
+    }
     if (maxRes < tol_feasOrg) use_feasOrg = 1;
     if (adjustSigmaYes) {
         lastSigmaIt = (double)it;
@@ -770,7 +831,8 @@
         double factor;
         adjust_lagrangian_param(sigma, resiPri / resiDual, factor);
         if (factor != 1.0) {
-            if (folded && rhs_valid && method != DOTSOCP_METHOD_ACCADMM) DS_CHECK(sigma_scale_folded(factor));
+            if (folded && rhs_valid && method != DOTSOCP_METHOD_ACCADMM) DS_CHECK(sigma_scale_folded(factor, pend));
+            else if (pend) { set_error("internal: a pending check without the folded sigma update"); return DOTSOCP_ESTATE; }
             else DS_CHECK(scale_state(1.0, factor, 1.0, true));
             if (method == DOTSOCP_METHOD_ACCADMM) DS_CHECK(acc_on_sigma_factor(factor));
         }
@@ -847,8 +909,11 @@
         timeout_pending = true;
         return 0;
     }
-    if (kkt_due || timed_out)
-        DS_CHECK(kkt_block(adjustSigmaYes, timed_out, brk, fold));
+    if (kkt_due || timed_out) {
+        const bool pend = fold && kkt_due && rhs_valid &&
+                          kkt_pend_form(it, opts.maxit, opts.ifCheckStepByStep != 0, last_of_run, timed_out, rescale, kkt_pend_eligible());
+        DS_CHECK(kkt_block(adjustSigmaYes, timed_out, brk, fold, pend));
+    }
     return 0;
 }
 
@@ -875,6 +940,7 @@
     }
     DS_CHECK(need_beta_form("the end of run()"));
     DS_CHECK(need_q("the end of run()"));
+    DS_CHECK(settle_pops());
     if (early_pass) { set_error("internal: an early cone pass is pending at the end of run()"); return DOTSOCP_ESTATE; }
     DS_CHECK(ensure_halo());
     DS_CHECK(sync_all());
diff --git a/include/dotsocp.h b/include/dotsocp.h
--- a/include/dotsocp.h
+++ b/include/dotsocp.h
@@ -125,6 +125,8 @@
 int dotsocp_rescale_due(dotsocp_i64 it, int rescale, double maxFeas, double relGap);
 int dotsocp_qcone_form(dotsocp_i64 it, double last_sigma_it, dotsocp_i64 maxit, int check_step_by_step, int last_of_run,
                        int next_last_of_run, int rescale, double maxFeas, double relGap);
+int dotsocp_kkt_pend_form(dotsocp_i64 it, dotsocp_i64 maxit, int check_step_by_step, int last_of_run, int timed_out,
+                          int rescale, int eligible);
 
 int dotsocp_upload(dotsocp_ctx *ctx, int field, const double *host);
 int dotsocp_download(dotsocp_ctx *ctx, int field, double *host);
```

Measured after the change: 100.5 (median of 6 runs). About the same (+1.1%).
